# empymod/emg3d

Measured on AMD Instinct MI355X. Metric: Mcells/s per multigrid cycle, higher is better.
Workload: dtype c128

## Files before the change

### emg3d_amd/_lib.py

```python
import ctypes
import os

import numpy as np

_HERE = os.path.dirname(os.path.abspath(__file__))
LIB_PATH = os.environ.get("EMG3D_HIP_LIB") or os.path.join(_HERE, "libemg3d_hip.so")
LAB_PATH = os.path.join(_HERE, "libemg3d_hip_lab.so")

c_i64 = ctypes.c_int64
c_int = ctypes.c_int
c_vp = ctypes.c_void_p
c_double = ctypes.c_double
c_dp = ctypes.POINTER(ctypes.c_double)

ABI_VERSION = 111

SIGNATURES = {
    "emg3d_hip_version": (c_int, []),
    "emg3d_hip_device_count": (c_int, [ctypes.POINTER(c_int)]),
    "emg3d_hip_set_device": (c_int, [c_int]),
    "emg3d_hip_device_info": (c_int, [c_int, ctypes.c_char_p, ctypes.POINTER(c_i64), ctypes.POINTER(c_int)]),
    "emg3d_hip_mem_info": (c_int, [c_int, ctypes.POINTER(c_i64), ctypes.POINTER(c_i64)]),
    "emg3d_hip_release_cached": (c_i64, []),
    "emg3d_hip_cached_bytes": (c_i64, []),
    "emg3d_hip_cached_bytes_on": (c_i64, [c_int]),
    "emg3d_mg_placement": (c_int, [c_vp, c_int, ctypes.POINTER(c_int), ctypes.POINTER(c_int), ctypes.POINTER(ctypes.c_float)]),
    "emg3d_amat_x": (c_int, [c_int, c_i64, c_i64, c_i64, c_vp, c_vp, c_vp, c_vp, c_vp, c_vp, c_vp, c_vp, c_vp]),
    "emg3d_get_h_field": (c_int, [c_int, c_i64, c_i64, c_i64, c_vp, c_vp, c_vp, c_vp, c_vp, c_vp, c_double, c_double]),
    "emg3d_gauss_seidel": (c_int, [c_int, c_int, c_i64, c_i64, c_i64, c_vp, c_vp, c_vp, c_vp, c_vp, c_vp,
                                   c_vp, c_vp, c_vp, c_int, c_int]),
    "emg3d_restrict": (c_int, [c_int, c_i64, c_i64, c_i64, c_i64, c_i64, c_i64, c_vp, c_vp, c_vp, c_int]),
    "emg3d_restrict_weights": (c_int, [c_vp, c_vp, c_vp, c_i64, c_vp, c_vp, c_vp, c_i64, c_vp, c_vp, c_vp]),
    "emg3d_solve": (c_int, [c_int, c_vp, c_vp, c_i64]),
    "emg3d_blocks_to_amat": (c_int, [c_int, c_vp, c_vp, c_i64, c_vp, c_vp, c_vp, c_i64, c_i64]),
    "emg3d_prolongation": (c_int, [c_int, c_i64, c_i64, c_i64, c_vp, c_vp, c_vp, c_vp, c_vp, c_vp, c_int]),
    "emg3d_restrict_model": (c_int, [c_int, c_i64, c_i64, c_i64, c_vp, c_vp, c_int]),
    "emg3d_sweep_plan": (c_int, [c_int, c_i64, c_i64, c_i64, c_int, c_int, c_int, c_int, ctypes.c_char_p, ctypes.POINTER(c_i64)]),
    "emg3d_sweep_fuse_plan": (c_int, [c_int, c_i64, c_i64, c_i64, c_int, c_int, c_int, c_int, c_int, c_int, c_int, c_i64, ctypes.POINTER(c_i64),
                                      ctypes.POINTER(c_i64), c_i64]),
    "emg3d_mg_create": (c_int, [ctypes.POINTER(c_vp), c_int, c_i64, c_i64, c_i64, c_vp, c_vp, c_vp, c_vp,
                                c_vp, c_vp, c_vp, c_vp, c_int]),
    "emg3d_mg_destroy": (None, [c_vp]),
    "emg3d_mg_create_sv": (c_int, [ctypes.POINTER(c_vp), c_int, c_i64, c_i64, c_i64, c_vp, c_vp, c_vp, c_vp,
                                   c_vp, c_vp, c_vp, c_vp, c_double, c_double, c_int]),
    "emg3d_mg_create_vs": (c_int, [ctypes.POINTER(c_vp), c_int, c_i64, c_i64, c_i64, c_vp, c_vp, c_vp, c_vp,
                                   c_vp, c_vp, c_vp, c_vp, c_vp, c_double, c_double, c_int, c_int]),
    "emg3d_mg_create_vse": (c_int, [ctypes.POINTER(c_vp), c_int, c_i64, c_i64, c_i64, c_vp, c_vp, c_vp, c_vp,
                                    c_vp, c_vp, c_vp, c_vp, c_vp, c_vp, c_double, c_double, c_double, c_int, c_int]),
    "emg3d_mg_set_smu0_eps": (c_int, [c_vp, c_double, c_double, c_double]),
    "emg3d_mg_set_model": (c_int, [c_vp, c_int, c_vp, c_vp, c_vp]),
    "emg3d_mg_get_sigma": (c_int, [c_vp, c_int, c_vp]),
    "emg3d_mg_set_sfield_vector": (c_int, [c_vp, c_vp, c_double, c_double]),
    "emg3d_mg_set_sfield_dipole": (c_int, [c_vp, c_vp, c_vp, c_int, c_int, c_vp]),
    "emg3d_source_field": (c_int, [c_int, c_i64, c_i64, c_i64, c_vp, c_vp, c_vp, c_vp, c_vp, c_vp, c_int, c_vp, c_vp]),
    "emg3d_mg_prepare": (c_int, [c_vp, c_int, c_int]),
    "emg3d_mg_set_trace": (c_int, [c_vp, c_int]),
    "emg3d_mg_get_trace": (c_int, [c_vp, c_int, c_vp, c_vp, c_vp]),
    "emg3d_mg_set_params": (c_int, [c_vp, c_int, c_int, c_int, c_int, c_int, c_vp, c_int]),
    "emg3d_mg_set_sfield": (c_int, [c_vp, c_vp]),
    "emg3d_mg_set_efield": (c_int, [c_vp, c_vp]),
    "emg3d_mg_get_efield": (c_int, [c_vp, c_vp]),
    "emg3d_mg_get_residual": (c_int, [c_vp, c_vp]),
    "emg3d_mg_get_hfield": (c_int, [c_vp, c_int, c_double, c_double, c_vp]),
    "emg3d_interp3d": (c_int, [c_int, c_i64, c_i64, c_i64, c_vp, c_vp, c_vp, c_vp, c_i64, c_vp, c_int, c_int, c_double,
                               c_double, c_vp]),
    "emg3d_get_receiver_response": (c_int, [c_int, c_i64, c_i64, c_i64, c_vp, c_vp, c_vp, c_vp, c_vp, c_int, c_i64,
                                            c_vp, c_vp, c_vp]),
    "emg3d_mg_get_receiver_response": (c_int, [c_vp, c_int, c_int, c_double, c_double, c_i64, c_vp, c_vp, c_vp]),
    "emg3d_edges2cellaverages": (c_int, [c_int, c_i64, c_i64, c_i64, c_vp, c_vp, c_vp, c_vp, c_vp]),
    "emg3d_mg_gradient": (c_int, [c_vp, c_int, c_double, c_double, c_vp]),
    "emg3d_mg_gradient3": (c_int, [c_vp, c_int, c_double, c_double, c_vp, c_vp, c_vp]),
    "emg3d_mg_grad_acc_reset": (c_int, [c_vp]),
    "emg3d_mg_grad_acc_add": (c_int, [c_vp, c_int, c_double, c_double, c_vp]),
    "emg3d_mg_grad_acc_get": (c_int, [c_vp, c_vp]),
    "emg3d_mg_grad_acc3_reset": (c_int, [c_vp]),
    "emg3d_mg_grad_acc3_add": (c_int, [c_vp, c_int, c_double, c_double, c_vp]),
    "emg3d_mg_grad_acc3_get": (c_int, [c_vp, c_vp, c_vp, c_vp]),
    "emg3d_cells2edges": (c_int, [c_int, c_i64, c_i64, c_i64, c_vp, c_vp, c_vp, c_vp, c_vp, c_vp, c_vp]),
    "emg3d_mg_jvec_source": (c_int, [c_vp, c_int, c_double, c_double, c_vp, c_vp, c_vp]),
    "emg3d_mg_jvec_source_b": (c_int, [c_vp, c_int, c_double, c_double, c_vp, c_vp, c_vp, c_vp]),
    "emg3d_mg_get_receiver_response_linear": (c_int, [c_vp, c_i64, c_vp, c_vp, c_vp]),
    "emg3d_mg_set_receiver_adjoint": (c_int, [c_vp, c_i64, c_vp, c_vp, c_vp, c_int]),
    "emg3d_mg_get_receiver_response_linear_h": (c_int, [c_vp, c_double, c_double, c_i64, c_vp, c_vp, c_vp]),
    "emg3d_mg_set_receiver_adjoint_ex": (c_int, [c_vp, c_int, c_int, c_double, c_double, c_i64, c_vp, c_vp, c_vp, c_int]),
    "emg3d_mg_set_receiver_adjoint_b": (c_int, [c_vp, c_int, c_int, c_double, c_double, c_i64, c_vp, c_vp, c_vp, c_vp, c_int]),
    "emg3d_receiver_adjoint": (c_int, [c_int, c_i64, c_i64, c_i64, c_vp, c_vp, c_vp, c_vp, c_int, c_int, c_double, c_double,
                                       c_i64, c_vp, c_vp, c_vp, c_vp]),
    "emg3d_volume_average_weights": (c_int, [c_vp, c_i64, c_vp, c_i64, c_vp, c_vp, c_vp, c_vp, c_vp]),
    "emg3d_volume_average": (c_int, [c_int, c_i64, c_i64, c_i64, c_vp, c_vp, c_vp, c_vp, c_i64, c_i64, c_i64, c_vp, c_vp,
                                     c_vp, c_vp, c_vp]),
    "emg3d_interp3d_grid": (c_int, [c_int, c_i64, c_i64, c_i64, c_vp, c_vp, c_vp, c_vp, c_i64, c_vp, c_i64, c_vp, c_i64,
                                    c_vp, c_int, c_int, c_double, c_double, c_vp]),
    "emg3d_mg_set_batch": (c_int, [c_vp, c_int]),
    "emg3d_mg_get_batch": (c_int, [c_vp]),
    "emg3d_mg_select": (c_int, [c_vp, c_int]),
    "emg3d_mg_set_mask": (c_int, [c_vp, c_vp]),
    "emg3d_mg_residual_norm": (c_int, [c_vp, c_dp]),
    "emg3d_mg_sfield_norm": (c_int, [c_vp, c_dp]),
    "emg3d_mg_smooth": (c_int, [c_vp, c_int, c_int]),
    "emg3d_mg_begin": (c_int, [c_vp, c_int]),
    "emg3d_mg_set_smu0": (c_int, [c_vp, ctypes.c_double, ctypes.c_double]),
    "emg3d_mg_cycle": (c_int, [c_vp, c_int, c_int, c_dp]),
    "emg3d_mg_cycle_next": (c_int, [c_vp, c_int, c_int, c_int, c_int, c_dp]),
    "emg3d_mg_cycles": (c_int, [c_vp, c_int, c_vp, c_int, c_vp, c_int, c_vp]),
    "emg3d_mg_efield_devptr": (c_vp, [c_vp]),
    "emg3d_mg_sfield_devptr": (c_vp, [c_vp]),
    "emg3d_mg_stream": (c_vp, [c_vp]),
    "emg3d_mg_nE": (c_i64, [c_vp]),
    "emg3d_mg_sync": (c_int, [c_vp]),
    "emg3d_mg_device_bytes": (c_i64, [c_vp]),
    "emg3d_mg_time_sweep": (c_int, [c_vp, c_int, c_int, ctypes.POINTER(ctypes.c_float)]),
    "emg3d_mg_last_sweep_kernel": (c_int, [c_vp, ctypes.c_char_p]),
    "emg3d_mg_time_residual": (c_int, [c_vp, c_int, ctypes.POINTER(ctypes.c_float)]),
    "emg3d_mg_last_residual_kernel": (c_int, [c_vp, ctypes.c_char_p]),
    "emg3d_mg_amatvec": (c_int, [c_vp, c_vp, c_vp]),
    "emg3d_mg_vec_alloc": (c_int, [c_vp, c_int]),
    "emg3d_mg_vec_set": (c_int, [c_vp, c_int, c_vp]),
    "emg3d_mg_vec_get": (c_int, [c_vp, c_int, c_vp]),
    "emg3d_mg_vec_copy": (c_int, [c_vp, c_int, c_int]),
    "emg3d_mg_vec_axpy": (c_int, [c_vp, c_int, c_double, c_double, c_int]),
    "emg3d_mg_vec_scale": (c_int, [c_vp, c_int, c_double, c_double]),
    "emg3d_mg_vec_dot": (c_int, [c_vp, c_int, c_int, c_dp]),
# ... 45 lines not shown


def load():
    global _lib, _path
    if _lib is None:
        _lib, _path = _open(LIB_PATH), LIB_PATH
    return _lib


def use(path=None):
    global _lib, _path
    prev = _path or LIB_PATH
    want = path or LIB_PATH
    _lib, _path = _open(want), want
    return prev


def check(status, what):
    if status != 0:
        raise HipLibraryError(f"{what} failed with status {status} "
                              f"({'invalid argument' if status < 0 else 'HIP error'})")


def dtype_code(dtype):
    dtype = np.dtype(dtype)
    if dtype == np.complex128:
        return 1
    if dtype == np.float64:
        return 0
    raise TypeError(f"fields must be float64 or complex128, got {dtype}")


def ptr(a):
    return a.ctypes.data_as(c_vp)


def device_count():
    n = c_int(0)
    check(load().emg3d_hip_device_count(ctypes.byref(n)), "emg3d_hip_device_count")
    return n.value


def device_info(device=0):
    name = ctypes.create_string_buffer(256)
    mem = c_i64(0)
    cus = c_int(0)
    check(load().emg3d_hip_device_info(device, name, ctypes.byref(mem), ctypes.byref(cus)),
          "emg3d_hip_device_info")
    return {"name": name.value.decode(), "total_mem": mem.value, "cu_count": cus.value}


def mem_info(device=0):
    fr, tot = c_i64(0), c_i64(0)
    check(load().emg3d_hip_mem_info(device, ctypes.byref(fr), ctypes.byref(tot)), "emg3d_hip_mem_info")
    return {"free": fr.value, "total": tot.value, "pooled": int(load().emg3d_hip_cached_bytes()),
            "pooled_on_device": int(load().emg3d_hip_cached_bytes_on(device))}


def sweep_plan(vnC, direction, dtype=np.complex128, ordering='colour', nsys=1, cu_count=0):
    name = ctypes.create_string_buffer(64)
    info = (c_i64 * 6)()
    check(load().emg3d_sweep_plan(dtype_code(dtype), int(vnC[0]), int(vnC[1]), int(vnC[2]), int(direction),
                                  1 if ordering == 'colour' else 0, int(nsys), int(cu_count), name, info), "emg3d_sweep_plan")
    return {"kernel": name.value.decode(), "lines_per_colour": info[0], "lines_per_wave": info[1], "rounds": info[2],
            "factor_kind": info[3], "split": bool(info[4]), "big_offsets": bool(info[5])}


def sweep_fuse_plan(vnC, direction, npass, dtype=np.complex128, ordering='colour', nsys=1, cu_count=0, own=0, max_seg=0, budget=0):
    info = (c_i64 * 8)()
    cap = (4 + 2 * max(int(npass), 0)) * (max(vnC) + 1)
    ranges = (c_i64 * cap)()
    check(load().emg3d_sweep_fuse_plan(dtype_code(dtype), int(vnC[0]), int(vnC[1]), int(vnC[2]), int(direction),
                                       1 if ordering == 'colour' else 0, int(nsys), int(cu_count), int(npass), int(own), int(max_seg), int(budget),
                                       info, ranges, cap), "emg3d_sweep_fuse_plan")
    out = {"fused": bool(info[0]), "axis": info[1], "nX": info[2], "own": info[3], "nslabs": info[4], "npass": info[5],
           "waves": info[6], "scratch_bytes": info[7], "slabs": []}
    if out["fused"]:
        per = 4 + 2 * int(npass)
        for k in range(info[4]):
            r = ranges[per * k:per * (k + 1)]
            out["slabs"].append({"own": (r[0], r[1]), "edges": (r[2], r[3]),
                                 "live": [(r[4 + 2 * p], r[5 + 2 * p]) for p in range(int(npass))]})
    return out
```

### emg3d_amd/csrc/emg3d_hip.hip

```cpp
#include "../../include/emg3d_hip.h"

#include <cstring>
#include <new>

#include <chrono>
#include "mg.hpp"
#include "receivers.hpp"
#include "source.hpp"
#include "gradient.hpp"
#include "regrid.hpp"

#define EMG3D_HIP_VERSION EMG3D_HIP_ABI_VERSION

namespace {

template <class T>
MG<T>* as(emg3d_mg_t* mg) { return static_cast<MG<T>*>(reinterpret_cast<emg3d_mg*>(mg)); }

static int current_device() { int d = 0; if (hipGetDevice(&d) != hipSuccess) { (void)hipGetLastError(); d = 0; } return d; }

template <class T> static T scalar_of(double re, double im);
template <> double scalar_of<double>(double re, double) { return re; }
template <> c128 scalar_of<c128>(double re, double im) { return mk(re, im); }

// ... 436 lines not shown
    std::vector<double> nodes[3], centers[3];
    for (int a = 0; a < 3; ++a) grid_vectors(hh[a], nC[a], origin ? origin[a] : 0.0, nodes[a], centers[a]);
    const i64 nF = is_electric ? n_edges(nC) : hfield_size(nC);
    T *df = nullptr, *scr = nullptr;
    DEV_ALLOC(df, (size_t)nF * sizeof(T));
    DEV_ALLOC(scr, (size_t)nF * sizeof(T));
    HIP_TRY(hipMemcpy(df, field, (size_t)nF * sizeof(T), hipMemcpyHostToDevice));
    RcvComp<T> comp[3];
    receiver_components<T>(nodes, centers, nC, is_electric != 0, df, comp);
    const int rc = receiver_response_device<T>(nullptr, comp, n, xyz, fac, scr, (T*)resp);
        return rc;
}

template <class T>
int interp3d_host_impl(i64 nx, i64 ny, i64 nz, const double* px, const double* py, const double* pz, const void* values,
                       i64 n, const double* xi, int method, int has_fill, double fill, double cval, void* out) {
    const i64 nn[3] = {nx, ny, nz};
    std::vector<double> pts[3];
    pts[0].assign(px, px + nx); pts[1].assign(py, py + ny); pts[2].assign(pz, pz + nz);
    const i64 tot = nx * ny * nz;
    T *dv = nullptr, *scr = nullptr, *dout = nullptr;
    DEV_ALLOC(dv, (size_t)tot * sizeof(T));
    DEV_ALLOC(scr, (size_t)tot * sizeof(T));
    DEV_ALLOC(dout, (size_t)n * sizeof(T));
    HIP_TRY(hipMemcpy(dv, values, (size_t)tot * sizeof(T), hipMemcpyHostToDevice));
    int rc = interp3d_device<T>(nullptr, dv, nn, 0, 1, nx, nx * ny, pts, n, xi, method, has_fill != 0, fill, cval, nullptr, scr, dout);
    if (rc == 0 && hipMemcpy(out, dout, (size_t)n * sizeof(T), hipMemcpyDeviceToHost) != hipSuccess) rc = (int)hipGetLastError();
        return rc;
}

}

template <class T>
static void* efield_ptr(MG<T>* m) {
    if (hipSetDevice(m->device) != hipSuccess) { (void)hipGetLastError(); return nullptr; }
    T* p = m->sel_e();
    m->check_launch();
    return m->err ? nullptr : (void*)p;
}

template <class T>
static int sweep_plan_impl(i64 nx, i64 ny, i64 nz, int dir, int order, int nsys, int cu_count, char* name, int64_t* info) {
    SweepKnobs K;
    if (cu_count > 0) K.simds = 4 * (i64)cu_count;
    else sweep_device_knobs<T>(K, current_device());
    K.order = order; K.nsys = nsys;
    const SweepPlan p = plan_sweep(K, SweepShape{{nx, ny, nz}, (int)sizeof(T)}, dir - 1);
    memcpy(name, p.name, sizeof p.name);
    info[0] = p.nmax; info[1] = p.lpw; info[2] = p.rounds; info[3] = p.fac_kind; info[4] = p.split ? 1 : 0; info[5] = p.big ? 1 : 0;
    return 0;
}

template <class T>
static int fuse_plan_impl(i64 nx, i64 ny, i64 nz, int dir, int order, int nsys, int cu_count, int npass, int own, int max_seg, i64 budget, int64_t* info,
                          int64_t* ranges, i64 nranges) {
    SweepKnobs K;
    if (cu_count > 0) K.simds = 4 * (i64)cu_count;
    else sweep_device_knobs<T>(K, current_device());
    K.order = order; K.nsys = nsys;
    if (own > 0) K.fuse_own = own;
    if (max_seg > 0) K.fuse_max_seg = max_seg;
    if (budget > 0) K.fuse_max_bytes = budget;
    const SweepShape G{{nx, ny, nz}, (int)sizeof(T)};
    const FusePlan f = plan_fuse(K, G, dir - 1, npass);
    int P, Q;
    sweep_axes(dir - 1, P, Q);
    info[0] = f.fused ? 1 : 0; info[1] = f.axis ? Q : P; info[2] = f.g.nX; info[3] = f.g.own; info[4] = f.g.nslabs; info[5] = f.g.npass;
    info[6] = f.nw; info[7] = f.scratch_bytes;
    if (!f.fused || !ranges) return 0;
    const i64 per = 4 + 2 * (i64)npass;
    if (nranges < per * f.g.nslabs) return -2;
    for (int k = 0; k < f.g.nslabs; ++k) {
        int64_t* r = ranges + per * k;
        r[0] = fuse_x0(f.g, k); r[1] = fuse_x1(f.g, k);
        i64 a = -1, b = -1;
        for (int j = 0; j <= f.g.nX; ++j) if (fuse_owner(f.g, j) == k) { if (a < 0) a = j; b = j + 1; }
        r[2] = a; r[3] = b;
        for (int p = 0; p < npass; ++p) { r[4 + 2 * p] = fuse_lo(f.g, k, p); r[5 + 2 * p] = fuse_hi(f.g, k, p); }
    }
    return 0;
}

template <class T>
static int jvec_stage(MG<T>* m, const double* const hv[3], const double* dv[3]) {
    Level<T>& L = *m->lv0;
    double* stage = reinterpret_cast<double*>(L.r);
    const i64 n = L.nCells;
    int used = 0;
    for (int c = 0; c < 3; ++c) {
        dv[c] = nullptr;
        if (!hv[c]) continue;
        for (int q = 0; q < c; ++q) if (hv[q] == hv[c]) dv[c] = dv[q];
        if (dv[c]) continue;
        double* d = stage + (i64)used++ * n;
        HIP_TRY(hipMemcpyAsync(d, hv[c], (size_t)n * sizeof(double), hipMemcpyHostToDevice, m->stream));
        dv[c] = d;
    }
    return 0;
}

template <class T>
static int jvec_source_impl(MG<T>* m, int efield_vec, double smu0_re, double smu0_im, const double* vx, const double* vy,
                            const double* vz) {
    if (sizeof(T) == 8 && smu0_im != 0.0) return -2;
    HIP_TRY(hipSetDevice(m->device));
    Level<T>& L = *m->lv0;
    const T* fwd = m->vec(efield_vec);
    if (!fwd || efield_vec < 0) return -2;
    const double* hv[3] = {vx, vy, vz};
    const double* dv[3];
    { const int st = jvec_stage<T>(m, hv, dv); if (st) return st; }
    T* s = m->sel_s();
    if (m->broken) return (int)hipErrorOutOfMemory;
    hipLaunchKernelGGL(k_jvec_source<T>, dim3((unsigned)((L.nE + 255) / 256)), dim3(256), 0, m->stream, L.nC[0], L.nC[1], L.nC[2],
                       L.fl, fwd, smu0_re, smu0_im, dv[0], dv[1], dv[2], (const double*)L.h[0], (const double*)L.h[1],
                       (const double*)L.h[2], s, L.nE);
    m->source_changed();
    m->lv0->s_dense = true;
    m->check_launch();
    return finish(m);
}

template <class T>
static int jvec_source_b_impl(MG<T>* m, int fwd_bvec, double smu0_re, double smu0_im, const double* vx, const double* vy,
                              const double* vz, const int32_t* use) {
    if (sizeof(T) == 8 && smu0_im != 0.0) return -2;
    HIP_TRY(hipSetDevice(m->device));
    Level<T>& L = *m->lv0;
    if (fwd_bvec < 0 || fwd_bvec >= (int)m->bvecs.size()) return -2;
    const T* fwd = m->bvecs[(size_t)fwd_bvec];
    unsigned long long bits = 0;
    for (int b = 0; b < m->nsys; ++b) if (use[b]) bits |= 1ull << b;
    if (!bits) return 0;
    const double* hv[3] = {vx, vy, vz};
    const double* dv[3];
    { const int st = jvec_stage<T>(m, hv, dv); if (st) return st; }
    if (m->broken) return (int)hipErrorOutOfMemory;
    hipLaunchKernelGGL(k_jvec_source_b<T>, dim3((unsigned)((L.nE + 255) / 256)), dim3(256), 0, m->stream, L.nC[0], L.nC[1], L.nC[2],
                       L.fl, fwd, m->nsys, bits, smu0_re, smu0_im, dv[0], dv[1], dv[2], (const double*)L.h[0], (const double*)L.h[1],
                       (const double*)L.h[2], L.s, L.nE);
    m->source_changed();
    m->lv0->s_dense = true;
    m->check_launch();
    return finish(m);
}

static int gradient_impl(emg3d_mg_t* mg, int efield_vec, double smu0_re, double smu0_im, double* gx, double* gy, double* gz) {
    const bool split = gy != nullptr;
    DISPATCH(mg, {
        HIP_TRY(hipSetDevice(m->device));
        Level<T>& L = *m->lv0;
        const T* fwd = m->vec(efield_vec);
        if (!fwd || efield_vec == -2) return -2;
        double* dg = reinterpret_cast<double*>(L.r);
        const i64 n = L.nCells;
        const unsigned blocks = (unsigned)((n + 255) / 256);
        const T* bwd = m->sel_e();
        if (m->broken) return (int)hipErrorOutOfMemory;
        if (split)
            hipLaunchKernelGGL((k_gradient<T, true>), dim3(blocks), dim3(256), 0, m->stream, L.nC[0], L.nC[1], L.nC[2], L.fl, fwd, bwd,
                               smu0_re, smu0_im, (const double*)L.h[0], (const double*)L.h[1], (const double*)L.h[2], dg, dg + n, dg + 2 * n);
        else
            hipLaunchKernelGGL((k_gradient<T, false>), dim3(blocks), dim3(256), 0, m->stream, L.nC[0], L.nC[1], L.nC[2], L.fl, fwd, bwd,
                               smu0_re, smu0_im, (const double*)L.h[0], (const double*)L.h[1], (const double*)L.h[2], dg, (double*)nullptr,
                               (double*)nullptr);
        m->check_launch();
// ... 171 lines not shown
    const hipError_t e = hipMemGetInfo(&fr, &tot);
    (void)hipSetDevice(prev);
    if (e != hipSuccess) { (void)hipGetLastError(); return (int)e; }
    if (free_bytes) *free_bytes = (int64_t)fr;
    if (total_bytes) *total_bytes = (int64_t)tot;
    return 0;
}

int emg3d_amat_x(int dtype, int64_t nx, int64_t ny, int64_t nz, void* r, const void* e, const void* eta_x,
                 const void* eta_y, const void* eta_z, const double* zeta, const double* hx,
                 const double* hy, const double* hz) {
    return dtype ? amat_x_impl<c128>(nx, ny, nz, r, e, eta_x, eta_y, eta_z, zeta, hx, hy, hz)
                 : amat_x_impl<double>(nx, ny, nz, r, e, eta_x, eta_y, eta_z, zeta, hx, hy, hz);
}

int emg3d_get_h_field(int dtype, int64_t nx, int64_t ny, int64_t nz, void* hfield, const void* efield,
                      const double* zeta, const double* hx, const double* hy, const double* hz,
                      double smu0_re, double smu0_im) {
    if (nx < 1 || ny < 1 || nz < 1 || !hfield || !efield || !hx || !hy || !hz) return -2;
    if (smu0_re == 0.0 && smu0_im == 0.0) return -2;
    if (!dtype && smu0_im != 0.0) return -2;
    return dtype ? hfield_impl<c128>(nx, ny, nz, hfield, efield, zeta, hx, hy, hz, smu0_re, smu0_im)
                 : hfield_impl<double>(nx, ny, nz, hfield, efield, zeta, hx, hy, hz, smu0_re, smu0_im);
}

int emg3d_gauss_seidel(int dtype, int dir, int64_t nx, int64_t ny, int64_t nz, void* e, const void* s,
                       const void* eta_x, const void* eta_y, const void* eta_z, const double* zeta,
                       const double* hx, const double* hy, const double* hz, int nu, int order) {
    return dtype ? gs_impl<c128>(dir, nx, ny, nz, e, s, eta_x, eta_y, eta_z, zeta, hx, hy, hz, nu, order)
                 : gs_impl<double>(dir, nx, ny, nz, e, s, eta_x, eta_y, eta_z, zeta, hx, hy, hz, nu, order);
}

int emg3d_restrict(int dtype, int64_t nx, int64_t ny, int64_t nz, int64_t cnx, int64_t cny, int64_t cnz,
                   void* cr, const void* r, const double* const* w, int sc_dir) {
    return dtype ? restrict_impl<c128>(nx, ny, nz, cnx, cny, cnz, cr, r, w, sc_dir)
                 : restrict_impl<double>(nx, ny, nz, cnx, cny, cnz, cr, r, w, sc_dir);
}

int emg3d_restrict_weights(const double* vectorN, const double* vectorCC, const double* h, int64_t nh,
                           const double* cvectorN, const double* cvectorCC, const double* ch, int64_t n,
                           double* wl, double* w0, double* wr) {
    if (n < 2 || nh < 2) return -2;
    restrict_weights_host(vectorN, vectorCC, h, nh, cvectorN, cvectorCC, ch, n, wl, w0, wr);
    return 0;
}

int emg3d_solve(int dtype, void* amat, void* bvec, int64_t n) {
    if (n < 1) return -2;
    return dtype ? solve_impl<c128>(amat, bvec, n) : solve_impl<double>(amat, bvec, n);
}

int emg3d_blocks_to_amat(int dtype, void* amat, void* bvec, int64_t n, const void* middle, const double* left,
                         const void* rhs, int64_t im, int64_t nC) {
    return dtype ? b2a_impl<c128>(amat, bvec, n, middle, left, rhs, im, nC)
                 : b2a_impl<double>(amat, bvec, n, middle, left, rhs, im, nC);
}

int emg3d_prolongation(int dtype, int64_t nx, int64_t ny, int64_t nz, const double* hx, const double* hy,
                       const double* hz, const double* origin, void* e, const void* ce, int sc_dir) {
    return dtype ? prolong_impl<c128>(nx, ny, nz, hx, hy, hz, origin, e, ce, sc_dir)
                 : prolong_impl<double>(nx, ny, nz, hx, hy, hz, origin, e, ce, sc_dir);
}

int emg3d_restrict_model(int is_complex, int64_t nx, int64_t ny, int64_t nz, void* cparam, const void* param,
                         int sc_dir) {
    return is_complex ? restrict_model_impl<c128>(nx, ny, nz, cparam, param, sc_dir)
                      : restrict_model_impl<double>(nx, ny, nz, cparam, param, sc_dir);
}

int emg3d_sweep_plan(int dtype, int64_t nx, int64_t ny, int64_t nz, int dir, int order, int nsys, int cu_count, char* name,
                     int64_t* info) {
    if (nx < 2 || ny < 2 || nz < 2 || dir < 1 || dir > 3 || order < 0 || order > 1 || nsys < 1 || nsys > 64 || !name || !info) return -2;
    return dtype ? sweep_plan_impl<c128>(nx, ny, nz, dir, order, nsys, cu_count, name, info)
                 : sweep_plan_impl<double>(nx, ny, nz, dir, order, nsys, cu_count, name, info);
}

int emg3d_sweep_fuse_plan(int dtype, int64_t nx, int64_t ny, int64_t nz, int dir, int order, int nsys, int cu_count, int npass, int own,
                          int max_seg, int64_t budget, int64_t* info, int64_t* ranges, int64_t nranges) {
    if (nx < 2 || ny < 2 || nz < 2 || dir < 1 || dir > 3 || order < 0 || order > 1 || nsys < 1 || nsys > 64 || npass < 0 || !info) return -2;
    return dtype ? fuse_plan_impl<c128>(nx, ny, nz, dir, order, nsys, cu_count, npass, own, max_seg, budget, info, ranges, nranges)
                 : fuse_plan_impl<double>(nx, ny, nz, dir, order, nsys, cu_count, npass, own, max_seg, budget, info, ranges, nranges);
}

int emg3d_mg_create(emg3d_mg_t** out, int dtype, int64_t nx, int64_t ny, int64_t nz, const double* hx,
                    const double* hy, const double* hz, const double* origin, const void* eta_x,
                    const void* eta_y, const void* eta_z, const double* zeta, int device) {
    if (!out) return -1;
    return dtype ? create_impl<c128>(out, 1, nx, ny, nz, hx, hy, hz, origin, eta_x, eta_y, eta_z, zeta, device)
                 : create_impl<double>(out, 0, nx, ny, nz, hx, hy, hz, origin, eta_x, eta_y, eta_z, zeta, device);
}

int emg3d_mg_create_sv(emg3d_mg_t** out, int dtype, int64_t nx, int64_t ny, int64_t nz, const double* hx,
                       const double* hy, const double* hz, const double* origin, const double* sv_x,
                       const double* sv_y, const double* sv_z, const double* zeta, double smu0_re,
                       double smu0_im, int device) {
    if (!out || !sv_x) return -1;
    return dtype ? create_impl<c128>(out, 1, nx, ny, nz, hx, hy, hz, origin, sv_x, sv_y, sv_z, zeta, device, true, smu0_re, smu0_im)
                 : create_impl<double>(out, 0, nx, ny, nz, hx, hy, hz, origin, sv_x, sv_y, sv_z, zeta, device, true, smu0_re, smu0_im);
}

int emg3d_mg_create_vs(emg3d_mg_t** out, int dtype, int64_t nx, int64_t ny, int64_t nz, const double* hx,
                       const double* hy, const double* hz, const double* origin, const double* sigma_x,
                       const double* sigma_y, const double* sigma_z, const double* vol, const double* zeta,
                       double smu0_re, double smu0_im, int map, int device) {
    if (!out || !sigma_x || !vol) return -1;
    if (map < 0 || map >= EMG_MAP_CODES) return -2;
    if (dtype ? smu0_re != 0.0 : smu0_im != 0.0) return -2;
    return dtype ? create_impl<c128>(out, 1, nx, ny, nz, hx, hy, hz, origin, sigma_x, sigma_y, sigma_z, zeta, device, true, smu0_re, smu0_im, vol, map)
                 : create_impl<double>(out, 0, nx, ny, nz, hx, hy, hz, origin, sigma_x, sigma_y, sigma_z, zeta, device, true, smu0_re, smu0_im, vol, map);
}

int emg3d_mg_create_vse(emg3d_mg_t** out, int dtype, int64_t nx, int64_t ny, int64_t nz, const double* hx,
                        const double* hy, const double* hz, const double* origin, const double* sigma_x,
                        const double* sigma_y, const double* sigma_z, const double* vol, const double* zeta,
                        const double* epsilon_r, double smu0_re, double smu0_im, double seps0, int map, int device) {
    if (!out || !sigma_x || !vol || !epsilon_r) return -1;
    if (map < 0 || map >= EMG_MAP_CODES) return -2;
    if (dtype ? smu0_re != 0.0 : smu0_im != 0.0) return -2;
    return dtype ? create_impl<c128>(out, 1, nx, ny, nz, hx, hy, hz, origin, sigma_x, sigma_y, sigma_z, zeta, device, true, smu0_re, smu0_im, vol, map, epsilon_r, seps0)
                 : create_impl<double>(out, 0, nx, ny, nz, hx, hy, hz, origin, sigma_x, sigma_y, sigma_z, zeta, device, true, smu0_re, smu0_im, vol, map, epsilon_r, seps0);
}

void emg3d_mg_destroy(emg3d_mg_t* mg) {
    if (!mg) return;
    const bool broken = reinterpret_cast<emg3d_mg*>(mg)->dtype ? as<c128>(mg)->broken : as<double>(mg)->broken;
    delete reinterpret_cast<emg3d_mg*>(mg);
    if (broken) (void)hipGetLastError();
}

int emg3d_mg_set_params(emg3d_mg_t* mg, int cycle, int nu_init, int nu_pre, int nu_coarse, int nu_post,
                        const int* clevel, int order) {
    if (cycle != 'V' && cycle != 'W' && cycle != 'F') return -2;
    if (order != 0 && order != 1) return -2;
    DISPATCH(mg, {
        bool same = m->cycle == cycle && m->nu_init == nu_init && m->nu_pre == nu_pre && m->nu_coarse == nu_coarse &&
                    m->nu_post == nu_post && m->order == order;
        if (clevel) for (int q = 0; q < 4; ++q) same = same && m->clevel[q] == clevel[q];
        if (!same) m->drop_graphs();
        m->cycle = cycle; m->cycmax = (cycle == 'V') ? 1 : 2;
        m->entry_cm = 0;
        m->nu_init = nu_init; m->nu_pre = nu_pre; m->nu_coarse = nu_coarse; m->nu_post = nu_post;
        if (clevel) {
            bool changed = false;
            for (int q = 0; q < 4; ++q) { if (m->clevel[q] != clevel[q]) changed = true; m->clevel[q] = clevel[q]; }
            if (changed) m->hier.clear();
        }
        if (m->order != order) {
            HIP_TRY(hipSetDevice(m->device));
            m->e_to_ref(*m->lv0);
            m->check_launch();
            m->order = order;
            m->forget_factors();
        }
        return 0;
    });
}

int emg3d_mg_set_smu0(emg3d_mg_t* mg, double smu0_re, double smu0_im) {
    DISPATCH(mg, {
        HIP_TRY(hipSetDevice(m->device));
        if (sizeof(T) == 8 && smu0_im != 0.0) return -2;
        if (sizeof(T) == 16 && m->volw && smu0_re != 0.0) return -2;
        if (m->epsr) return -7;
        const int st = m->set_smu0(scalar_of<T>(smu0_re, smu0_im));
        if (st) return st;
        return finish(m);
// ... 690 lines not shown
```

### emg3d_amd/csrc/mg.hpp

```cpp
#pragma once
#include <algorithm>
#include <cmath>
#include <cstdlib>
#include <cstring>
#include <map>
#include <memory>
#include <mutex>
#include <chrono>
#include <vector>

#include "common.hpp"
#include "smooth.hpp"
#include "stencil.hpp"
#include "gradient.hpp"
#include "smooth_qpl.hpp"
#include "smooth_qc.hpp"
#include "smooth_thm.hpp"
#include "smooth_tha.hpp"
#include "sweep_launch.hpp"
#include "sweep_plan.hpp"

template <class T>
struct Level {
    i64 nC[3];
    i64 nE, nCells;
    FieldLayout fl;
    CellLayout cl;
    std::vector<double> h_host[3], nodes[3], centers[3];
    double* h[3] = {nullptr, nullptr, nullptr};
    double* ih[3] = {nullptr, nullptr, nullptr};
    T* eta[3] = {nullptr, nullptr, nullptr};
    double* zeta = nullptr;
    unsigned char* sflag[3] = {nullptr, nullptr, nullptr};
    bool sflag_valid[3] = {false, false, false};
    bool s_dense = false;
    bool zeta_sep = false;
    T *s = nullptr, *e = nullptr, *r = nullptr;
    T *eT = nullptr, *sT = nullptr;
    T* etaT[3] = {nullptr, nullptr, nullptr};
    double* zetaT = nullptr;
    bool sT_valid = false;
    FieldLayout flT;
    CellLayout clT;
    T *eW[2] = {nullptr, nullptr}, *sW[2] = {nullptr, nullptr};
    double* zetaW[2] = {nullptr, nullptr};
    bool sW_valid[2] = {false, false};
    int e_home = 0;
    T* fac[3] = {nullptr, nullptr, nullptr};
    void* qd[3][4] = {{nullptr, nullptr, nullptr, nullptr}, {nullptr, nullptr, nullptr, nullptr}, {nullptr, nullptr, nullptr, nullptr}};
    unsigned qdn[3][4] = {{0, 0, 0, 0}, {0, 0, 0, 0}, {0, 0, 0, 0}};
    T* fz[3] = {nullptr, nullptr, nullptr};
    i64 fz_n[3] = {0, 0, 0};
    FusePlan fuse[3];
    int fuse_key[3] = {-1, -1, -1};
    std::vector<int> passes[3];
    i64 fac_lines[3] = {0, 0, 0};
    i64 fac_mid[3] = {0, 0, 0};
    int fac_kind[3] = {0, 0, 0};
    SweepPlan plan[3];
    int plan_key[3] = {-1, -1, -1};
};

struct Transfer {
    int sc = -1;
    int co[3] = {0, 0, 0};
    double* w[3][3] = {{nullptr, nullptr, nullptr}, {nullptr, nullptr, nullptr}, {nullptr, nullptr, nullptr}};
    int* pidx[3] = {nullptr, nullptr, nullptr};
    double* pwt[3] = {nullptr, nullptr, nullptr};
};

template <class T>
struct Hierarchy {
    std::vector<std::shared_ptr<Level<T>>> lv;
    std::vector<Transfer> tr;
};

class DevicePool {
    std::mutex mu;
    struct Parked { void* p; int tag; };
    std::multimap<std::pair<int, size_t>, Parked> free_blocks;
    size_t held = 0, cap;
public:
    DevicePool() {
        const char* g = getenv("EMG3D_POOL_GB");
        cap = (size_t)((g ? atof(g) : 96.0) * (double)((size_t)1 << 30));
    }
    void* take(int device, size_t nb, int tag = 0, bool* hit = nullptr) {
        std::lock_guard<std::mutex> lk(mu);
        if (hit) *hit = false;
        auto rng = free_blocks.equal_range({device, nb});
        if (rng.first == rng.second) return nullptr;
        auto pick = rng.second;
        for (auto it = rng.first; it != rng.second; ++it) if (it->second.tag == tag) { pick = it; break; }
        if (pick == rng.second && tag != 0)
            for (auto it = rng.first; it != rng.second; ++it) if (it->second.tag == 0) { pick = it; break; }
        if (pick == rng.second) pick = rng.first;
        if (hit) *hit = tag != 0 && pick->second.tag == tag;
        void* p = pick->second.p;
        free_blocks.erase(pick);
        held -= nb;
        return p;
    }
    bool give(int device, void* p, size_t nb, int tag = 0) {
        std::lock_guard<std::mutex> lk(mu);
        if (held + nb > cap) return false;
        free_blocks.insert({{device, nb}, Parked{p, tag}});
        held += nb;
        return true;
    }
    size_t release_all() {
        std::lock_guard<std::mutex> lk(mu);
        const size_t n = held;
        int cur = 0;
        (void)hipGetDevice(&cur);
        for (auto& kv : free_blocks) {
            if (kv.first.first < 0) { (void)hipHostFree(kv.second.p); continue; }
            (void)hipSetDevice(kv.first.first); (void)hipFree(kv.second.p);
        }
        for (auto& kv : free_streams) { (void)hipSetDevice(kv.first); (void)hipStreamDestroy(kv.second); }
        free_streams.clear();
        (void)hipSetDevice(cur);
        free_blocks.clear();
        held = 0;
        return n;
    }
    size_t bytes_held() { std::lock_guard<std::mutex> lk(mu); return held; }
    size_t bytes_held_on(int device) {
        std::lock_guard<std::mutex> lk(mu);
        size_t n = 0;
        for (auto& kv : free_blocks) if (kv.first.first == device) n += kv.first.second;
        return n;
    }
    std::multimap<int, hipStream_t> free_streams;
    hipStream_t take_stream(int device) {
        {
// ... 915 lines not shown
                a.rs.off[c] = (unsigned)a.fl.off[ax[c]];
                for (int d = 0; d < 3; ++d) a.rs.st[c][d] = (unsigned)a.fl.st[ax[c]][ax[d]];
            }
        }
        a.qd = nullptr; a.qdn = 0;
        a.fe = nullptr; a.fnE = 0; a.fax = a.fnX = a.fown = a.fns = a.fnp = 0; a.fseq = 0;
        for (int c = 0; c < 4; ++c) { a.fqd[c] = nullptr; a.fqdn[c] = 0; }
        a.qpl = P.NW; a.qM = P.M; a.seg = P.seg; a.qlpw = 0;
        a.tha = P.helpers;
        a.mode = 0; a.cP = a.cQ = 0; a.cntA = a.cntB = 0; a.t = a.jQ0 = a.cnt = 0;
        a.bt = sweep ? batch(L) : Batch();
    }

    void ensure_factor(Level<T>& L, int dir) {
        const SweepPlan& P = plan(L, dir);
        if (P.xt) ensure_transposed_model(L);
        if (L.fac[dir]) return;
        L.fac_lines[dir] = (L.nC[dir == 0 ? 1 : 0] - 1) * (L.nC[dir == 2 ? 1 : 2] - 1);
        L.fac[dir] = dalloc<T>(L.fac_lines[dir] * P.fac_entries);
        L.fac_mid[dir] = P.mid;
        L.fac_kind[dir] = P.fac_kind;
        if (P.fac_kind == 3) thm_attrs();
        compute_factor(L, dir);
    }
    void compute_factor(Level<T>& L, int dir) {
        LineArgs<T> a;
        line_args(L, dir, a, false);
        a.fac = L.fac[dir];
        a.fcomp = L.fac_kind[dir] == 4;
        if (L.fac_kind[dir] == 3) {
            a.mid = L.fac_mid[dir];
            const i64 nQ_ = L.nC[a.Q];
            const i64 nmax_ = a.nA[0] * ((nQ_ - 0) / 2);
            a.mode = 3;
            if (nmax_ > 0)
                MG_LAUNCH(k_line_factor_m<T>, dim3((unsigned)((nmax_ + EMG_LINE_BLOCK - 1) / EMG_LINE_BLOCK), 4),
                                   dim3(EMG_LINE_BLOCK), 0, stream, a);
            check_launch();
            return;
        }
        a.mid = L.fac_mid[dir];
        const i64 nQ = L.nC[a.Q];
        const i64 nB[2] = {(nQ - 0) / 2, (nQ - 1) / 2};
        a.mode = 3; a.cP = a.cQ = 0; a.cntA = a.cntB = 0;
        const i64 nmax = a.nA[0] * nB[0];
#ifdef EMG3D_LAB
        if (LAB_ENV("EMG3D_FACTOR_PER_COLOUR", 0)) {
            for (int c = 0; c < 4; ++c) {
                a.mode = 0; a.cP = c & 1; a.cQ = c >> 1; a.cntA = a.nA[a.cP]; a.cntB = nB[a.cQ];
                const i64 n = a.cntA * a.cntB;
                if (n > 0)
                    MG_LAUNCH(k_line_factor<T>, dim3((unsigned)((n + EMG_LINE_BLOCK - 1) / EMG_LINE_BLOCK)),
                                       dim3(EMG_LINE_BLOCK), 0, stream, a);
            }
            check_launch();
            return;
        }
#endif
        if (nmax > 0)
            MG_LAUNCH(k_line_factor<T>, dim3((unsigned)((nmax + EMG_LINE_BLOCK - 1) / EMG_LINE_BLOCK), 4),
                               dim3(EMG_LINE_BLOCK), 0, stream, a);
        check_launch();
    }

    unsigned xcd_grid(i64 nb) const { return (unsigned)(xcd_map ? ((nb + 7) / 8) * 8 : nb); }
    unsigned rp_grid(i64 nt) const { return xcd_grid((nt + EMG_RP_BLOCK - 1) / EMG_RP_BLOCK); }
    void ensure_qdesc(Level<T>& L, int dir) {
        const SweepPlan& P = plan(L, dir);
        if (!P.qdesc || L.qd[dir][0] || L.qdn[dir][0] == ~0u) return;
        L.qdn[dir][0] = ~0u;
        if (!L.fac[dir]) return;
        LineArgs<T> a;
        line_args(L, dir, a, true);
        const i64 lpg = 16 / a.seg;
        a.bt = Batch();
        for (int c = 0; c < 4; ++c) {
            a.mode = 0; a.cP = c & 1; a.cQ = c >> 1;
            a.cntA = a.nA[a.cP]; a.cntB = a.nB2[a.cQ];
            a.rs.slot0 = (unsigned)a.base[c];
            const i64 n = a.cntA * a.cntB;
            if (n <= 0) continue;
            const unsigned grid = xcd_grid((n + lpg - 1) / lpg);
            const i64 nthreads = (i64)grid * 64;
            void* tab = try_alloc<char>(nthreads * a.qM * (3 * 16 + 8 * 16));
            if (!tab) return;
            a.qd = tab; a.qdn = (unsigned)nthreads;
            if (!broken) qpl_launch<T>(1, a.qM, false, 1, false, dim3(grid), stream, a);
            L.qd[dir][c] = tab; L.qdn[dir][c] = (unsigned)nthreads;
        }
        check_launch();
    }
    char sweep_name[64] = "";
    char res_name[64] = "";
    int thm_lifo = (int)LAB_ENV("EMG3D_THM_LIFO", 0);
    void thm_attrs() {
#ifdef EMG3D_LAB
        static bool done[64] = {false};
        if (device < 0 || device >= 64 || done[device]) return;
        done[device] = true;
        thm_lifo_attrs<T>();
#endif
    }
    void launch_sweep(const SweepPlan& P, const LineArgs<T>& a, i64 n) {
        if (log_launches) fprintf(stderr, "[sweep] nC %lld %lld %lld L %d lines %lld kernel %s split %d\n", (long long)a.nC[0], (long long)a.nC[1], (long long)a.nC[2], a.L, (long long)n,
                                  P.name, a.split);
        memcpy(sweep_name, P.name, sizeof sweep_name);
        if (broken) return;
        switch (P.family) {
        case SweepFamily::tha: {
            const size_t dyn = P.helpers == 2 ? tha_lds_bytes<T, 2>((int)a.nC[a.L]) : tha_lds_bytes<T, 3>((int)a.nC[a.L]);
            tha_launch<T>(P.helpers, a.zsep != 0, bgrid(xcd_grid((n + THA_LPW - 1) / THA_LPW)), dyn, stream, a);
            break;
        }
        case SweepFamily::thm: {
            const i64 npairs = (n + P.inst_lpw - 1) / P.inst_lpw;
            thm_launch<T>(P.stages, P.inst_lpw, thm_lifo != 0, a.zsep != 0, bgrid(rp_grid(npairs * 128)), stream, a);
            break;
        }
        case SweepFamily::qpl:
        case SweepFamily::qpl_chain: {
            const i64 lpg = (16 * P.NW) / P.seg;
            qpl_launch<T>(P.NW, P.M, false, (P.NW == 1 && a.qd) ? 2 : 0, P.family == SweepFamily::qpl_chain,
                          bgrid(xcd_grid((n + lpg - 1) / lpg)), stream, a);
            break;
        }
        case SweepFamily::qc:
        case SweepFamily::qc_big: {
            LineArgs<T> b = a;
            b.qlpw = P.inst_lpw == 16 ? sweep_balanced_lpw(knobs, n * nsys) : P.inst_lpw;
            qc_launch<T>(P.stages, P.inst_lpw, a.zsep != 0, P.big, bgrid(rp_grid(((n + b.qlpw - 1) / b.qlpw) * 64)), stream, b);
            break;
        }
        case SweepFamily::rp: {
            const unsigned g = rp_grid(((n + P.inst_lpw - 1) / P.inst_lpw) * 64);
            if (P.inst_lpw == 8) hipLaunchKernelGGL((k_line_sweep_rp<T, 8>), bgrid(g), dim3(EMG_RP_BLOCK), 0, stream, a);
            else if (P.inst_lpw == 12) hipLaunchKernelGGL((k_line_sweep_rp<T, 12>), bgrid(g), dim3(EMG_RP_BLOCK), 0, stream, a);
            else hipLaunchKernelGGL((k_line_sweep_rp<T, 4>), bgrid(g), dim3(EMG_RP_BLOCK), 0, stream, a);
            break;
        }
        case SweepFamily::tpl:
            hipLaunchKernelGGL(k_line_sweep<T>, bgrid_y((unsigned)((n + EMG_LINE_BLOCK - 1) / EMG_LINE_BLOCK)), dim3(EMG_LINE_BLOCK), 0, stream, a);
            break;
        }
    }

    void prepare_work(Level<T>& L, int dir) {
        ensure_sflags(L, dir);
        if (home_on(L) || home_lvl(L)) ensure_work(L, 1);
        if (split_on(L)) ensure_work(L, (dir == 0) ? 0 : 1);
        else if (plan(L, dir).xt) ensure_transposed_model(L);
    }
    void to_work(Level<T>& L, int dir) {
        ensure_sflags(L, dir);
        if (split_on(L)) {
            const int w = (dir == 0) ? 0 : 1;
            ensure_work(L, w);
            if (home_lvl(L)) {
                if (w == 0) {
                    if (!L.sW_valid[0]) { convert_field(L, L.sW[0], L.sW[1], 2, true); L.sW_valid[0] = true; }
                    convert_field(L, L.eW[0], L.eW[1], 2, true);
                }
                return;
            }
            if (!L.sW_valid[w]) { convert_field(L, L.sW[w], L.s, w, true); L.sW_valid[w] = true; }
            if (!home_on(L)) convert_field(L, L.eW[w], L.e, w, true);
            else {
                e_to_w1(L);
// ... 69 lines not shown
            if (placed[w] || dir < 0 || !L.eW[w] || !L.sW[w] || !L.fac[dir]) continue;
            placed[w] = true;
            if (w == 1) e_to_ref(L);
            if (!L.sW_valid[w]) { convert_field(L, L.sW[w], L.s, w, true); L.sW_valid[w] = true; }
            ensure_sflags(L, dir);
            const i64 n = (i64)nsys * L.nE;
            PlaceRec& R = place_rec[w];
            R = PlaceRec();
            T* cands[PLACE_MAX];
            cands[0] = L.eW[w];
            int best = 0;
            float worst = 0.f;
            const int nt = std::min<int>(place_tries, PLACE_MAX);
            for (int k = 0; k < nt; ++k) {
                T* c = (k == 0) ? cands[0] : try_alloc<T>(n);
                if (!c) break;
                cands[k] = c;
                hipMemsetAsync(c, 0, (size_t)n * sizeof(T), stream);
                L.eW[w] = c;
                if (k == 0) (void)time_sweeps(L, dir, 1);
                const float ms = time_sweeps(L, dir, place_reps);
                R.ms[k] = ms;
                R.tries = k + 1;
                if (ms < 0.f) break;
                if (ms < R.ms[best]) best = k;
                worst = std::max(worst, ms);
                if ((double)R.ms[best] * place_gap < (double)worst) break;
            }
            if (R.ms[best] < 0.f) best = 0;
            R.kept = best;
            L.eW[w] = cands[best];
            block_tag[cands[best]] = 1 + w;
            for (int k = 0; k < R.tries; ++k) if (k != best) release(cands[k]);
            moved |= best != 0;
            if (getenv("EMG3D_LOG_SETUP")) {
                fprintf(stderr, "[place] working copy %d (%s-lines, %.0f MB): kept candidate %d of %d;", w, dir == 0 ? "x" : dir == 1 ? "y" : "z",
                        (double)n * sizeof(T) / 1048576.0, best, R.tries);
                for (int k = 0; k < R.tries; ++k) fprintf(stderr, " %.3f", R.ms[k]);
                fprintf(stderr, " ms per sweep\n");
            }
        }
        if (moved) drop_graphs();
        check_launch();
    }

    void colour_passes(Level<T>& L, int dir, int nu, std::vector<int>& seq) {
        int Pa, Qa;
        sweep_axes(dir, Pa, Qa);
        const i64 nP = L.nC[Pa], nQ = L.nC[Qa];
        int iback = 0, last_c = -1;
        seq.clear();
        for (int it = 0; it < nu; ++it) {
            iback = 1 - iback;
            for (int ch = 0; ch < 4; ++ch) {
                const int c = iback ? colour_perm_b[ch] : colour_perm[ch];
                if (skip_idempotent && c == last_c) continue;
                last_c = c;
                if (((nP - (c & 1)) / 2) * ((nQ - (c >> 1)) / 2) <= 0) continue;
                seq.push_back(c);
            }
        }
    }
    const FusePlan& ensure_fuse(Level<T>& L, int dir, int nu) {
        const int key = nu * 256 + order + 2 * nsys;
        if (L.fuse_key[dir] == key) return L.fuse[dir];
        FusePlan& F = L.fuse[dir];
        F = FusePlan();
        L.fuse_key[dir] = key;
        L.passes[dir].clear();
        if (order != 1) return F;
        colour_passes(L, dir, nu, L.passes[dir]);
        const std::vector<int>& seq = L.passes[dir];
        plan(L, dir);
        F = plan_fuse(knobs, SweepShape{{L.nC[0], L.nC[1], L.nC[2]}, (int)sizeof(T)}, dir, (int)seq.size());
        if (!F.fused) return F;
        for (int c : seq) if (!L.qd[dir][c]) { F.fused = false; return F; }
        const i64 need = (i64)nsys * F.g.nslabs * L.nE;
        if (L.fz_n[dir] < need) {
            T* z = try_alloc<T>(need);
            if (!z) { F.fused = false; return F; }
            if (L.fz[dir]) release(L.fz[dir]);
            L.fz[dir] = z; L.fz_n[dir] = need;
        }
        return F;
    }
    void smooth_fused(Level<T>& L, int dir, const SweepPlan& P, const FusePlan& F, const std::vector<int>& seq, const LineArgs<T>& a) {
        LineArgs<T> b = a;
        b.mode = 0; b.xcd = 0;
        b.fe = L.fz[dir]; b.fnE = L.nE; b.fax = F.axis;
        b.fnX = F.g.nX; b.fown = F.g.own; b.fns = F.g.nslabs; b.fnp = F.g.npass;
        b.fseq = 0;
        for (int p = 0; p < F.g.npass; ++p) b.fseq |= (unsigned long long)seq[(size_t)p] << (4 * p);
        for (int c = 0; c < 4; ++c) { b.fqd[c] = L.qd[dir][c]; b.fqdn[c] = L.qd[dir][c] ? L.qdn[dir][c] : 0u; }
        if (log_launches) fprintf(stderr, "[sweep] nC %lld %lld %lld L %d lines %lld kernel %s split %d fused passes %d slabs %d own %d\n", (long long)a.nC[0],
                                  (long long)a.nC[1], (long long)a.nC[2], a.L, (long long)a.nLinesTot, P.name, a.split, F.g.npass, F.g.nslabs, F.g.own);
        memcpy(sweep_name, P.name, sizeof sweep_name);
        if (broken) return;
        qpl_fused_launch<T>(P.family == SweepFamily::qpl_chain, bgrid((unsigned)F.g.nslabs), stream, b);
        ScatterArgs sa;
        sa.nE = L.nE; sa.g = F.g;
        int Pa, Qa;
        sweep_axes(dir, Pa, Qa);
        sa.ax = F.axis ? Qa : Pa;
        for (int c = 0; c < 3; ++c) {
            sa.off[c] = L.fl.off[c];
            sa.d0[c] = (unsigned)((c == 0) ? L.nC[0] : L.nC[0] + 1); sa.d1[c] = (unsigned)((c == 1) ? L.nC[1] : L.nC[1] + 1);
        }
        hipLaunchKernelGGL(k_scatter_slabs<T>, dim3((unsigned)((L.nE + EMG_BLOCK - 1) / EMG_BLOCK), (unsigned)nsys), dim3(EMG_BLOCK), 0, stream,
                           a.e, (const T*)L.fz[dir], sa, a.bt);
    }

    void smooth_line(Level<T>& L, int dir, int nu, bool conv_in = true, bool conv_out = true) {
        if (nu <= 0) return;
        ensure_factor(L, dir);
        ensure_qdesc(L, dir);
        const FusePlan& F = ensure_fuse(L, dir, nu);
        if (dry) { prepare_work(L, dir); return; }
        if (conv_in) to_work(L, dir);
        ensure_sflags(L, dir);
        LineArgs<T> a;
        line_args(L, dir, a, true);
        const SweepPlan& P = plan(L, dir);
        const i64 nP = L.nC[a.P], nQ = L.nC[a.Q];
        const i64 nB[2] = {(nQ - 0) / 2, (nQ - 1) / 2};
        if (order == 1) {
            if (F.fused) smooth_fused(L, dir, P, F, L.passes[dir], a);
            else for (int c : L.passes[dir]) {
                a.mode = 0; a.cP = c & 1; a.cQ = c >> 1;
                a.cntA = a.nA[a.cP]; a.cntB = nB[a.cQ];
                a.rs.slot0 = (unsigned)a.base[c];
                a.qd = L.qd[dir][c]; a.qdn = (L.qd[dir][c] ? L.qdn[dir][c] : 0u);
                launch_sweep(P, a, a.cntA * a.cntB);
            }
            nu = 0;
        }
        int iback = 0;
        for (int it = 0; it < nu; ++it) {
            iback = 1 - iback;
            {
                const i64 tmin = 3, tmax = (nP - 1) + 2 * (nQ - 1);
                if (lex_loop && a.qpl && a.qM == 1 && a.seg <= 16) {
                    LineArgs<T> b = a;
                    b.mode = 2; b.t = tmin; b.jQ0 = tmax; b.cnt = iback; b.xcd = 0;
                    const i64 maxn = std::min<i64>(nQ - 1, (nP - 1) / 2 + 1), quads = maxn * a.seg;
                    const int lnw = quads <= 16 ? 1 : quads <= 32 ? 2 : quads <= 64 ? 4 : 8;
                    if (!broken) qpl_launch<T>(lnw, 1, true, 0, false, bgrid(1), stream, b);
                    sweep_kernel_name(sweep_name, sizeof sweep_name, SweepFamily::qpl, (int)sizeof(T), lnw, 1);
                    continue;
                }
                for (i64 th = tmin; th <= tmax; ++th) {
                    const i64 tt = iback ? tmax - (th - tmin) : th;
                    i64 lo = tt - (nP - 1);
                    i64 jQ0 = lo <= 0 ? 1 : (lo + 1) / 2;
                    if (jQ0 < 1) jQ0 = 1;
                    i64 jQ1 = (tt - 1) / 2;
                    if (jQ1 > nQ - 1) jQ1 = nQ - 1;
                    const i64 n = jQ1 - jQ0 + 1;
                    if (n <= 0) continue;
                    a.mode = 1; a.t = tt; a.jQ0 = jQ0; a.cnt = n;
                    launch_sweep(P, a, n);
                }
            }
        }
        if (conv_out) from_work(L, dir);
        check_launch();
    }

    void smooth_point(Level<T>& L, int nu) {
        if (dry) return;
        if (&L == lv0.get()) e_to_ref(L);
        const bool hl = home_lvl(L) && L.e_home == 1;
        if (hl) { convert_field(L, L.e, L.eW[1], 1, false); convert_field(L, L.s, L.sW[1], 1, false); }
        PointArgs<T> a;
        for (int q = 0; q < 3; ++q) { a.nC[q] = L.nC[q]; a.eta[q] = L.eta[q]; a.h[q] = L.h[q]; a.ih[q] = L.ih[q]; }
        a.fl = L.fl; a.e = L.e; a.s = L.s; a.zeta = L.zeta; a.bt = batch(L);
        a.col = 0; a.t = 0; a.cnt[0] = a.cnt[1] = a.cnt[2] = 0;
        int iback = 0;
        int last_c = -1;
        for (int it = 0; it < nu; ++it) {
            iback = 1 - iback;
            if (order == 1) {
// ... 162 lines not shown
        Level<T>& L = *lv0;
        if (L.sT && !L.sT_valid) { convert_field(L, L.sT, L.s, -1, true); L.sT_valid = true; }
        for (int w = 0; w < 2; ++w)
            if (L.sW[w] && !L.sW_valid[w]) { convert_field(L, L.sW[w], L.s, w, true); L.sW_valid[w] = true; }
        for (int d = 0; d < 3; ++d)
            if (L.sflag[d]) ensure_sflags(L, d);
    }

    void prepare(int g, int lr_dir) {
        if (!use_graph) { dry = true; cycle0_eager(g, lr_dir, 0); dry = false; place_level0(lr_dir); return; }
        cycle0(g, lr_dir, -1);
    }

    void cycle0(int g, int lr_dir, int slot) {
        if (!use_graph || trace) {
            if (slot >= 0) {
                if (placement_pending(lr_dir)) prepare(g, lr_dir);
                cycle0_eager(g, lr_dir, slot);
            }
            return;
        }
        const int key = (g * 8 + lr_dir) * 4 + entry_cm;
        auto it = graphs.find(key);
        if (it != graphs.end() && slot < 0) return;
        const int home_in = (home_on(*lv0) && current_lr_dir(lr_dir, lv0->nC) != 0) ? 1 : 0;
        if (it == graphs.end()) {
            const bool tlog = getenv("EMG3D_LOG_SETUP") != nullptr;
            auto now = [] { return std::chrono::steady_clock::now(); };
            auto ms = [](auto a, auto b) { return std::chrono::duration<double, std::milli>(b - a).count(); };
            auto t0 = now();
            const size_t nalloc0 = allocs.size();
            dry = true;
            cycle0_eager(g, lr_dir, 0);
            dry = false;
            place_level0(lr_dir);
            const int home_keep = (slot >= 0) ? home_in : lv0->e_home;
            if (slot >= 0) { if (home_in) e_to_w1(*lv0); else e_to_ref(*lv0); }
            else if (home_in) ensure_work(*lv0, 1);
            lv0->e_home = home_in;
            refresh_level0_source();
            if (tlog) hipStreamSynchronize(stream);
            auto t1 = now();
            hipGraph_t graph = nullptr;
            hipGraphExec_t exec = nullptr;
            hipError_t st = hipStreamBeginCapture(stream, hipStreamCaptureModeThreadLocal);
            if (st == hipSuccess) {
                cycle0_eager(g, lr_dir, 0);
                st = hipStreamEndCapture(stream, &graph);
            }
            const int home_out = lv0->e_home;
            lv0->e_home = home_keep;
            auto t2 = now();
            if (st == hipSuccess) st = hipGraphInstantiate(&exec, graph, nullptr, nullptr, 0);
            if (graph) hipGraphDestroy(graph);
            if (tlog) fprintf(stderr, "[setup] key %d: hierarchy+factors %.2f ms (%zu allocations), capture %.2f ms, instantiate %.2f ms\n",
                              key, ms(t0, t1), allocs.size() - nalloc0, ms(t1, t2), ms(t2, now()));
            if (st != hipSuccess || err != 0) {
                (void)hipGetLastError();
                fprintf(stderr, "[emg3d_hip] hipGraph capture failed (%s); using eager launches\n", hipGetErrorString(st));
                use_graph = false;
                err = 0;
                if (slot >= 0) cycle0_eager(g, lr_dir, slot);
                return;
            }
            (void)hipGraphUpload(exec, stream);
            graphs[key] = exec;
            graph_home[key] = std::make_pair(home_in, home_out);
            it = graphs.find(key);
            if (slot < 0) return;
        }
        const std::pair<int, int> hm = graph_home[key];
        if (hm.first) e_to_w1(*lv0); else e_to_ref(*lv0);
        refresh_level0_source();
        hipError_t st = hipGraphLaunch(it->second, stream);
        if (st != hipSuccess && err == 0) err = (int)st;
        lv0->e_home = hm.second;
        if (slot != 0) hipMemcpyAsync(norms + (i64)slot * nsys, norms, (size_t)nsys * sizeof(double), hipMemcpyDeviceToDevice, stream);
    }

    void forget_factors() {
        auto clear = [](Level<T>& L) {
            for (int d = 0; d < 3; ++d) {
                L.fac[d] = nullptr; L.fac_kind[d] = 0; L.plan_key[d] = -1; L.fuse_key[d] = -1;
                for (int c = 0; c < 4; ++c) { L.qd[d][c] = nullptr; L.qdn[d][c] = 0; }
            }
        };
        if (lv0) clear(*lv0);
        for (auto& kv : hier) for (auto& l : kv.second.lv) if (l) clear(*l);
    }

    void drop_graphs() {
        for (auto& kv : graphs) hipGraphExecDestroy(kv.second);
        graphs.clear();
        graph_home.clear();
        graph_seen.clear();
    }
};
```

### emg3d_amd/csrc/smooth.hpp

```cpp
#pragma once
#include "common.hpp"

#define EMG_LINE_BLOCK 64

template <class T>
struct LineArgs {
    int L, P, Q;
    i64 nC[3];
    FieldLayout fl;
    CellLayout cl;
    T* e;
    const T* s;
    const T* eta[3];
    const double* zeta;
    const double* h[3];
    const double* ih[3];
    int split;
    i64 mid;
    int xcd;
    int tile;
    struct Resolved {
        const double *ihL, *ihP, *ihQ;
        const double *hL, *hP, *hQ;
        unsigned nL, csL, csP, csQ;
        unsigned nP, nQ;
        unsigned slot0;
        unsigned off[3], st[3][3];
    } rs;
    Batch bt;
    int qm;
    int qpl;
    int qM, seg;
    const unsigned char* sflag;
    int zsep;
    int qlpw;
    int tha;
    int fcomp;
    T* fac;
    const void* qd;
    unsigned qdn;
    T* fe;
    i64 fnE;
    int fax, fnX, fown, fns, fnp;
    unsigned long long fseq;
    const void* fqd[4];
    unsigned fqdn[4];
    i64 nLinesTot;
    i64 base[4];
    i64 nA[2];
    i64 nB2[2];
    int mode;
    int cP, cQ;
    i64 cntA, cntB;
    i64 t, jQ0, cnt;
};

template <class T>
__device__ __forceinline__ bool line_of_thread(const LineArgs<T>& a, i64& jP, i64& jQ) {
    const i64 idx = (i64)blockIdx.x * blockDim.x + threadIdx.x;
    if (a.mode == 0) {
        if (idx >= a.cntA * a.cntB) return false;
        const i64 b = idx / a.cntA, q = idx - b * a.cntA;
        jP = 1 + a.cP + 2 * q;
        jQ = 1 + a.cQ + 2 * b;
    } else {
        if (idx >= a.cnt) return false;
        jQ = a.jQ0 + idx;
        jP = a.t - 2 * jQ;
    }
    return true;
}

template <class T>
__device__ __forceinline__ i64 line_slot(const LineArgs<T>& a, i64 jP, i64 jQ) {
    const int cP = (int)((jP - 1) & 1), cQ = (int)((jQ - 1) & 1);
    return a.base[cP + 2 * cQ] + ((jP - 1) >> 1) + a.nA[cP] * ((jQ - 1) >> 1);
}

struct LineCoef {
    double QP_Lm[2], PQ_Lm[2];
    double QL_Pm[2], LQ_Pm[2], QL_Pp[2], LQ_Pp[2];
    double PL_Qm[2], LP_Qm[2], PL_Qp[2], LP_Qp[2];
};

__device__ __forceinline__ void line_coef(LineCoef& c, const double z[2][2][2], const double kL[2],
                                          const double kP[2], const double kQ[2]) {
#pragma unroll
    for (int S = 0; S < 2; ++S) {
        c.QP_Lm[S] = kP[S] * (z[0][S][1] + z[0][S][0]);
        c.PQ_Lm[S] = kQ[S] * (z[0][1][S] + z[0][0][S]);
        c.QL_Pm[S] = kL[S] * (z[S][0][1] + z[S][0][0]);
        c.LQ_Pm[S] = kQ[S] * (z[1][0][S] + z[0][0][S]);
        c.QL_Pp[S] = kL[S] * (z[S][1][1] + z[S][1][0]);
        c.LQ_Pp[S] = kQ[S] * (z[1][1][S] + z[0][1][S]);
        c.PL_Qm[S] = kL[S] * (z[S][1][0] + z[S][0][0]);
        c.LP_Qm[S] = kP[S] * (z[1][S][0] + z[0][S][0]);
        c.PL_Qp[S] = kL[S] * (z[S][1][1] + z[S][0][1]);
        c.LP_Qp[S] = kP[S] * (z[1][S][1] + z[0][S][1]);
    }
}

__device__ __forceinline__ void line_left(const LineCoef& c, double ihLm, double a[5], double d[5]) {
    a[0] = 0.0; d[0] = 0.0;
    a[1] = c.QP_Lm[0] * ihLm;
    a[2] = -c.QP_Lm[1] * ihLm;
    a[3] = c.PQ_Lm[0] * ihLm;
    a[4] = -c.PQ_Lm[1] * ihLm;
    d[1] = -c.QL_Pm[0] * ihLm;
    d[2] = -c.QL_Pp[0] * ihLm;
    d[3] = -c.PL_Qm[0] * ihLm;
    d[4] = -c.PL_Qp[0] * ihLm;
}

__host__ __device__ __forceinline__ constexpr int wpk(int r, int c) {
    return r >= c ? r * (r + 1) / 2 + c : c * (c + 1) / 2 + r;
}

template <class T>
__device__ __forceinline__ void apply_sinv(const T f[15], T y[5]) {
    T o[5];
#pragma unroll
    for (int r = 0; r < 5; ++r) {
        T t = f[wpk(r, 0)] * y[0];
#pragma unroll
        for (int c = 1; c < 5; ++c) t += f[wpk(r, c)] * y[c];
        o[r] = t;
    }
#pragma unroll
    for (int r = 0; r < 5; ++r) y[r] = o[r];
}

template <class T>
struct BlockMat {
    T S[5][5];
    double al[5], dl[5];
};

template <class T>
// ... 1092 lines not shown
```

### emg3d_amd/csrc/smooth_qpl.hpp

```cpp
#pragma once
#include "smooth.hpp"
#include "sweep_plan.hpp"


template <int K>
__device__ __forceinline__ double quad_bcast(double v) {
    constexpr int ctrl = K | (K << 2) | (K << 4) | (K << 6);
    int lo = __double2loint(v), hi = __double2hiint(v);
    lo = __builtin_amdgcn_update_dpp(0, lo, ctrl, 0xf, 0xf, false);
    hi = __builtin_amdgcn_update_dpp(0, hi, ctrl, 0xf, 0xf, false);
    return __hiloint2double(hi, lo);
}
template <int K>
__device__ __forceinline__ c128 quad_bcast(c128 v) { return mk(quad_bcast<K>(v.re), quad_bcast<K>(v.im)); }
__device__ __forceinline__ double quad_sum(double v) {
    int lo = __double2loint(v), hi = __double2hiint(v);
    double o = __hiloint2double(__builtin_amdgcn_update_dpp(0, hi, 0xb1, 0xf, 0xf, false),
                                __builtin_amdgcn_update_dpp(0, lo, 0xb1, 0xf, 0xf, false));
    v += o;
    lo = __double2loint(v); hi = __double2hiint(v);
    o = __hiloint2double(__builtin_amdgcn_update_dpp(0, hi, 0x4e, 0xf, 0xf, false),
                         __builtin_amdgcn_update_dpp(0, lo, 0x4e, 0xf, 0xf, false));
    return v + o;
}
__device__ __forceinline__ c128 quad_sum(c128 v) { return mk(quad_sum(v.re), quad_sum(v.im)); }

template <bool UP>
__device__ __forceinline__ double row_shift4(double v) {
    constexpr int ctrl = UP ? 0x114 : 0x104;
    int lo = __double2loint(v), hi = __double2hiint(v);
    lo = __builtin_amdgcn_update_dpp(0, lo, ctrl, 0xf, 0xf, false);
    hi = __builtin_amdgcn_update_dpp(0, hi, ctrl, 0xf, 0xf, false);
    return __hiloint2double(hi, lo);
}
template <bool UP> __device__ __forceinline__ c128 row_shift4(c128 v) { return mk(row_shift4<UP>(v.re), row_shift4<UP>(v.im)); }
template <bool UP> __device__ __forceinline__ double lane_shift4(double v) { return UP ? __shfl_up(v, 4) : __shfl_down(v, 4); }
template <bool UP> __device__ __forceinline__ c128 lane_shift4(c128 v) { return mk(lane_shift4<UP>(v.re), lane_shift4<UP>(v.im)); }

template <class T>
__device__ __forceinline__ void qpl_args_burst(const LineArgs<T>& a) {
    asm volatile("" :: "s"(a.e), "s"(a.s), "s"(a.fac), "s"(a.zeta), "s"(a.rs.ihL), "s"(a.rs.ihP), "s"(a.rs.ihQ), "s"(a.bt.st),
                 "s"(a.bt.mask), "s"(a.bt.n), "s"(a.xcd), "s"(a.mode), "s"(a.cntA), "s"(a.cntB), "s"(a.cP), "s"(a.cQ), "s"(a.seg),
                 "s"(a.rs.nL), "s"(a.rs.csL), "s"(a.rs.csP), "s"(a.rs.csQ), "s"(a.rs.slot0), "s"(a.rs.off[0]), "s"(a.rs.off[1]),
                 "s"(a.rs.off[2]));
    asm volatile("" :: "s"(a.rs.st[0][0]), "s"(a.rs.st[0][1]), "s"(a.rs.st[0][2]), "s"(a.rs.st[1][0]), "s"(a.rs.st[1][1]),
                 "s"(a.rs.st[1][2]), "s"(a.rs.st[2][0]), "s"(a.rs.st[2][1]), "s"(a.rs.st[2][2]), "s"(a.t), "s"(a.jQ0), "s"(a.cnt),
                 "s"(a.rs.nP), "s"(a.rs.nQ), "s"(a.qd), "s"(a.qdn));
}

template <class T, int NW, int M, bool HL = false, int DM = 0, bool CH = false, bool FZ = false>
__global__ __launch_bounds__(64 * NW) void k_line_sweep_qpl(LineArgs<T> a) {
    static_assert(DM == 0 || (!HL && (NW == 1 || FZ)), "descriptors: one wave per workgroup, colour order");
    static_assert(!CH || ((NW == 1 || FZ) && M == 1 && !HL), "chain form: lines inside one wave, one block per quad");
    static_assert(!FZ || (DM == 2 && M == 1 && !HL), "fused passes: descriptors, one block per quad, colour order");
    constexpr int NQ = 16 * NW;
#ifdef EMG3D_LAB
    long long qts[7] = {0, 0, 0, 0, 0, 0, 0};
#define QPL_TS(i) do { if (a.tile & 512) { asm volatile("" ::: "memory"); qts[i] = (long long)__builtin_readcyclecounter(); asm volatile("" ::: "memory"); } } while (0)
#else
#define QPL_TS(i) do {} while (0)
#endif
    QPL_TS(0);
    qpl_args_burst(a);
    QPL_TS(1);
    const int tid = threadIdx.x;
    const int quad = tid >> 2, r = tid & 3;
    const int seg = a.seg;
    const int ch = quad & (seg - 1);
    const int lseg = __builtin_ctz((unsigned)seg);
    const int lpg = NQ >> lseg;
    typedef unsigned int u32;
    EMG_SWEEP_WG(a)
    __shared__ T xb[2][(FZ && CH) ? 1 : NQ][4][5];
    T* const ebase = FZ ? a.fe + ((i64)bsys_ * a.fns + wg) * a.fnE : a.e + boff_;
    const void* qd_ = a.qd;
    u32 qdn_ = a.qdn;
    u32 tix = (u32)wg * (64u * NW) + (u32)tid;
    auto one = [&](const u32 gline, const u32 nlines, const u32 t_, const u32 jQ0_) {
    const bool live = gline < nlines;
    const int nL = (int)a.rs.nL;
    auto ld_d = [](const double* base, u32 idx) -> double { return *reinterpret_cast<const double*>(reinterpret_cast<const char*>(base) + idx * 8u); };
    auto ld_t = [](const T* base, u32 idx) -> T { return *reinterpret_cast<const T*>(reinterpret_cast<const char*>(base) + idx * (u32)sizeof(T)); };
    const T* __restrict__ e = ebase;
    const T* __restrict__ s = (a.s + boff_);
    T Wr[M][5], W0[M][5];
    T b[M][5];
    double av[M][4], dv[M][4];
    bool lastb[M], inl[M];
    u32 dS[M], dS0[M];
    constexpr int QD_U4 = 3, QD_D2 = 8;
    if constexpr (DM == 2) {
        const uint4* const q4 = reinterpret_cast<const uint4*>(qd_);
        const emg_d2* const c2 = reinterpret_cast<const emg_d2*>(q4 + (size_t)(QD_U4 * M) * qdn_);
        uint4 u[M][QD_U4];
        emg_d2 cf[M][QD_D2];
#pragma unroll
        for (int j = 0; j < M; ++j) {
#pragma unroll
            for (int k = 0; k < QD_U4; ++k) u[j][k] = q4[(u32)(QD_U4 * j + k) * qdn_ + tix];
#pragma unroll
            for (int k = 0; k < QD_D2; ++k) cf[j][k] = c2[(u32)(QD_D2 * j + k) * qdn_ + tix];
        }
        QPL_TS(2);
        T E[M][6], S[M], E0[M], S0[M];
#pragma unroll
        for (int j = 0; j < M; ++j) {
            const u32 oE[6] = {u[j][0].x, u[j][0].y, u[j][0].z, u[j][0].w, u[j][1].x, u[j][1].y};
            dS[j] = u[j][1].z; dS0[j] = u[j][2].x;
            inl[j] = (u[j][2].z & 1u) != 0; lastb[j] = (u[j][2].z & 2u) != 0;
            const T* w = a.fac + u[j][2].y;
#pragma unroll
            for (int c = 0; c < 5; ++c) W0[j][c] = w[(u32)(wpk(0, c) * (M * seg))];
#pragma unroll
            for (int c = 0; c < 5; ++c) {
                const int e1 = wpk(1, c), e2 = wpk(2, c), e3 = wpk(3, c), e4 = wpk(4, c);
                const int en = (r == 0) ? e1 : (r == 1) ? e2 : (r == 2) ? e3 : e4;
                Wr[j][c] = w[(u32)(en * (M * seg))];
            }
#pragma unroll
            for (int t = 0; t < 6; ++t) E[j][t] = ld_t(e, oE[t]);
            S[j] = ld_t(s, dS[j]);
            E0[j] = ld_t(e, u[j][1].w);
            S0[j] = ld_t(s, dS0[j]);
        }
#pragma unroll
        for (int j = 0; j < M; ++j) {
            const double cE[6] = {cf[j][0].x, cf[j][0].y, cf[j][1].x, cf[j][1].y, cf[j][2].x, cf[j][2].y};
            av[j][0] = cf[j][3].y; av[j][1] = cf[j][4].x; av[j][2] = cf[j][4].y; av[j][3] = cf[j][5].x;
            dv[j][0] = cf[j][5].y; dv[j][1] = cf[j][6].x; dv[j][2] = cf[j][6].y; dv[j][3] = cf[j][7].x;
            T y = S[j];
#pragma unroll
            for (int t = 0; t < 6; ++t) cmac(y, E[j][t], cE[t]);
            const T bo = lastb[j] ? Zero<T>::v() : y;
            T part = E0[j] * cf[j][3].x;
            part = quad_sum(part);
            b[j][0] = S0[j] + part;
            b[j][1] = quad_bcast<0>(bo); b[j][2] = quad_bcast<1>(bo); b[j][3] = quad_bcast<2>(bo); b[j][4] = quad_bcast<3>(bo);
            if (!inl[j]) {
#pragma unroll
                for (int c = 0; c < 5; ++c) { Wr[j][c] = Zero<T>::v(); W0[j][c] = Zero<T>::v(); }
            }
        }
    } else {
    const u32 gidx = live ? gline : 0u;
    u32 jP, jQ;
    if (a.mode == 0) {
        const u32 cA = (u32)a.cntA;
        const u32 bq = gidx / cA, qq = gidx - bq * cA;
        jP = 1u + (u32)a.cP + 2u * qq;
        jQ = 1u + (u32)a.cQ + 2u * bq;
    } else {
        jQ = jQ0_ + gidx;
        jP = t_ - 2u * jQ;
    }
    const u32 slot = (a.mode == 0) ? a.rs.slot0 + gidx : (u32)line_slot(a, (i64)jP, (i64)jQ);
    const u32 csL = a.rs.csL, csP = a.rs.csP, csQ = a.rs.csQ;
    const double ihP[2] = {ld_d(a.rs.ihP, jP - 1u), ld_d(a.rs.ihP, jP)};
    const double ihQ[2] = {ld_d(a.rs.ihQ, jQ - 1u), ld_d(a.rs.ihQ, jQ)};
    const bool tp = r < 2;
    const int side = r & 1;
    const double sg = side ? -1.0 : 1.0;
    const u32 jA = tp ? jP : jQ, jB = tp ? jQ : jP;
    const u32 acell = jA - 1u + (u32)side;
    const u32 anode = side ? jA + 1u : jA - 1u;
    const u32 oLc = a.rs.off[0], oAc = tp ? a.rs.off[1] : a.rs.off[2], oBc = tp ? a.rs.off[2] : a.rs.off[1];
    const u32 sLL = a.rs.st[0][0];
    const u32 sLA = tp ? a.rs.st[0][1] : a.rs.st[0][2], sLB = tp ? a.rs.st[0][2] : a.rs.st[0][1];
    const u32 sAL = tp ? a.rs.st[1][0] : a.rs.st[2][0];
    const u32 sAA = tp ? a.rs.st[1][1] : a.rs.st[2][2], sAB = tp ? a.rs.st[1][2] : a.rs.st[2][1];
    const u32 sBL = tp ? a.rs.st[2][0] : a.rs.st[1][0];
    const u32 sBA = tp ? a.rs.st[2][1] : a.rs.st[1][2], sBB = tp ? a.rs.st[2][2] : a.rs.st[1][1];
    u32 ob[7], os[7];
    ob[0] = oAc + sAL + acell * sAA + jB * sAB;
    ob[1] = oLc + sLL + anode * sLA + jB * sLB;
    ob[2] = ob[1] - sLL;
    ob[3] = oBc + sBL + anode * sBA + jB * sBB;
    ob[4] = ob[3] - sBB;
    ob[5] = ob[0] + sAB;
    ob[6] = ob[0] - sAB;
    os[0] = sAL; os[1] = sLL; os[2] = sLL; os[3] = sBL; os[4] = sBL; os[5] = sAL; os[6] = sAL;
    const u32 sLP = a.rs.st[0][1], sLQ = a.rs.st[0][2];
    const u32 o0 = oLc + jP * sLP + jQ * sLQ;
    const u32 db0 = (r < 2) ? sLP : sLQ;
    const u32 ob0 = (r & 1) ? o0 - db0 : o0 + db0;
    const int type = tp ? 1 : 2;

    T E[M][6], S[M], E0[M], S0[M];
    u32 dE[M][6], dE0[M], dF[M];
    double f00[M], f10[M], f01[M], f11[M], n0[M], n1[M], ihl0[M], ihl1[M];
#pragma unroll
    for (int j = 0; j < M; ++j) {
        const int i = ch * M + j;
        const int ic = i < nL ? i : nL - 1;
        inl[j] = i < nL;
        lastb[j] = (ic == nL - 1);
        if constexpr (DM == 0) {
            const T* w = a.fac + ((i64)slot * (15 * (M * seg)) + ic);
#pragma unroll
            for (int c = 0; c < 5; ++c) W0[j][c] = w[(u32)(wpk(0, c) * (M * seg))];
#pragma unroll
            for (int c = 0; c < 5; ++c) {
                const int e1 = wpk(1, c), e2 = wpk(2, c), e3 = wpk(3, c), e4 = wpk(4, c);
                const int en = (r == 0) ? e1 : (r == 1) ? e2 : (r == 2) ? e3 : e4;
                Wr[j][c] = w[(u32)(en * (M * seg))];
            }
        } else {
// ... 123 lines not shown
            for (int cc = 0; cc < 4; ++cc) {
                T t = g0 * oG[0][cc];
                cmac(t, g1, oG[1][cc]); cmac(t, g2, oG[2][cc]); cmac(t, g3, oG[3][cc]);
                mG[cc] = t;
            }
        }
    };
    auto compose_c_only = [&](int p, int src) {
        cmac(mc, mG[0], xb[p][src][0][0]); cmac(mc, mG[1], xb[p][src][1][0]);
        cmac(mc, mG[2], xb[p][src][2][0]); cmac(mc, mG[3], xb[p][src][3][0]);
    };
    int p = 0;

    auto fwd_row = [&](int j) {
        T t = Wr[j][0] * b[j][0];
#pragma unroll
        for (int c = 1; c < 5; ++c) cmac(t, Wr[j][c], b[j][c]);
        mc = t;
#pragma unroll
        for (int k = 0; k < 4; ++k) {
            T g = Zero<T>::v();
            cmsc(g, Wr[j][0], av[j][k]);
            cmsc(g, Wr[j][k + 1], dv[j][k]);
            mG[k] = g;
        }
    };
    fwd_row(0);
    T u[4];
    if constexpr (CH) {
        auto from_below = [&](T v) -> T { return seg == 4 ? row_shift4<true>(v) : lane_shift4<true>(v); };
        T zc = mc;
#pragma unroll 1
        for (int st = 1; st < seg; ++st) {
            const T up = from_below(zc);
            T t0 = mc, t1 = mG[1] * quad_bcast<1>(up);
            cmac(t0, mG[0], quad_bcast<0>(up)); cmac(t1, mG[3], quad_bcast<3>(up)); cmac(t0, mG[2], quad_bcast<2>(up));
            zc = (ch > 0) ? t0 + t1 : mc;
        }
        const T up = from_below(zc);
        u[0] = quad_bcast<0>(up); u[1] = quad_bcast<1>(up); u[2] = quad_bcast<2>(up); u[3] = quad_bcast<3>(up);
        if (ch == 0) { u[0] = Zero<T>::v(); u[1] = Zero<T>::v(); u[2] = Zero<T>::v(); u[3] = Zero<T>::v(); }
    } else {
#pragma unroll
    for (int j = 1; j < M; ++j) {
        publish(p);
        sync();
        fwd_row(j);
        compose_with(p, quad);
        p ^= 1;
    }
#pragma unroll 1
    for (int st = 1; st < seg; st <<= 1) {
        publish(p);
        sync();
        if (ch >= st) { if (2 * st < seg) compose_with(p, quad - st); else compose_c_only(p, quad - st); }
        p ^= 1;
    }
    publish(p);
    sync();
#pragma unroll
    for (int k = 0; k < 4; ++k) u[k] = (ch > 0) ? xb[p][quad - 1][k][0] : Zero<T>::v();
    p ^= 1;
    }
    T z0[M], zr[M];
#pragma unroll
    for (int j = 0; j < M; ++j) {
        T y[5];
        y[0] = b[j][0];
#pragma unroll
        for (int k = 0; k < 4; ++k) {
            cmsc(y[0], u[k], av[j][k]);
            T t = b[j][k + 1];
            cmsc(t, u[k], dv[j][k]);
            y[k + 1] = t;
        }
        z0[j] = W0[j][0] * y[0];
        zr[j] = Wr[j][0] * y[0];
#pragma unroll
        for (int c = 1; c < 5; ++c) { cmac(z0[j], W0[j][c], y[c]); cmac(zr[j], Wr[j][c], y[c]); }
        if (j + 1 < M) { u[0] = quad_bcast<0>(zr[j]); u[1] = quad_bcast<1>(zr[j]); u[2] = quad_bcast<2>(zr[j]); u[3] = quad_bcast<3>(zr[j]); }
    }

    QPL_TS(4);
    auto bwd_row = [&](int j) {
        const double ar = (r == 0) ? av[j][0] : (r == 1) ? av[j][1] : (r == 2) ? av[j][2] : av[j][3];
        const double dr = (r == 0) ? dv[j][0] : (r == 1) ? dv[j][1] : (r == 2) ? dv[j][2] : dv[j][3];
        T g = z0[j] * ar;
        cmac(g, zr[j], dr);
        mc = g;
#pragma unroll
        for (int l = 0; l < 4; ++l) {
            T h = Zero<T>::v();
            cmsc(h, W0[j][l + 1], ar);
            cmsc(h, Wr[j][l + 1], dr);
            mG[l] = h;
        }
    };
    bwd_row(M - 1);
    T v[4];
    if constexpr (CH) {
        auto from_above = [&](T w) -> T { return seg == 4 ? row_shift4<false>(w) : lane_shift4<false>(w); };
        T vc = mc;
        const bool inner = ch + 1 < seg;
#pragma unroll 1
        for (int st = 1; st < seg; ++st) {
            const T dn = from_above(vc);
            T t0 = mc, t1 = mG[1] * quad_bcast<1>(dn);
            cmac(t0, mG[0], quad_bcast<0>(dn)); cmac(t1, mG[3], quad_bcast<3>(dn)); cmac(t0, mG[2], quad_bcast<2>(dn));
            vc = inner ? t0 + t1 : mc;
        }
        const T dn = from_above(vc);
        v[0] = quad_bcast<0>(dn); v[1] = quad_bcast<1>(dn); v[2] = quad_bcast<2>(dn); v[3] = quad_bcast<3>(dn);
        if (!inner) { v[0] = Zero<T>::v(); v[1] = Zero<T>::v(); v[2] = Zero<T>::v(); v[3] = Zero<T>::v(); }
    } else {
#pragma unroll
    for (int j = M - 2; j >= 0; --j) {
        publish(p);
        sync();
        bwd_row(j);
        compose_with(p, quad);
        p ^= 1;
    }
#pragma unroll 1
    for (int st = 1; st < seg; st <<= 1) {
        publish(p);
        sync();
        if (ch + st < seg) { if (2 * st < seg) compose_with(p, quad + st); else compose_c_only(p, quad + st); }
        p ^= 1;
    }
    publish(p);
    sync();
#pragma unroll
    for (int k = 0; k < 4; ++k) v[k] = (ch + 1 < seg) ? xb[p][quad + 1][k][0] : Zero<T>::v();
    }
    QPL_TS(5);
    T* eo = ebase;
#pragma unroll
    for (int j = M - 1; j >= 0; --j) {
        T x0 = z0[j], xr = zr[j];
#pragma unroll
        for (int l = 0; l < 4; ++l) { cmsc(x0, W0[j][l + 1], v[l]); cmsc(xr, Wr[j][l + 1], v[l]); }
        const int i = ch * M + j;
        if (live && inl[j]) {
            if (r == 0) eo[dS0[j]] = x0;
            if (!lastb[j]) eo[dS[j]] = xr;
        }
        if (j > 0) {
            const double ar = (r == 0) ? av[j][0] : (r == 1) ? av[j][1] : (r == 2) ? av[j][2] : av[j][3];
            const double dr = (r == 0) ? dv[j][0] : (r == 1) ? dv[j][1] : (r == 2) ? dv[j][2] : dv[j][3];
            T vr = x0 * ar;
            cmac(vr, xr, dr);
            v[0] = quad_bcast<0>(vr); v[1] = quad_bcast<1>(vr); v[2] = quad_bcast<2>(vr); v[3] = quad_bcast<3>(vr);
        }
    }
    QPL_TS(6);
    };

    if constexpr (FZ) {
        const FuseGeom g{a.fnX, a.fown, a.fns, a.fnp};
        const int k = (int)wg;
        {
            T* __restrict__ dst = ebase;
            const T* __restrict__ src = a.e + boff_;
            const int ra = fuse_lo(g, k, 0) - 1, rb = fuse_hi(g, k, 0) + 1;
            const int X = a.fax ? 2 : 1;
            const u32 nO = a.fax ? a.rs.nP : a.rs.nQ;
#pragma unroll
            for (int c = 0; c < 3; ++c) {
                const u32 dL = a.rs.nL + (c != 0 ? 1u : 0u), dX = (u32)g.nX + (c != X ? 1u : 0u), dO = nO + ((c == 0 || c == X) ? 1u : 0u);
                const int rbc = rb < (int)dX - 1 ? rb : (int)dX - 1;
                if (rbc < ra) continue;
                const u32 w = (u32)(rbc - ra + 1);
                const u32 stL = a.rs.st[c][0], stX = a.fax ? a.rs.st[c][2] : a.rs.st[c][1], stO = a.fax ? a.rs.st[c][1] : a.rs.st[c][2];
                const bool xf = stX < stL;
                const u32 n0 = xf ? w : dL, n1 = xf ? dL : w, tot = n0 * n1 * dO;
                for (u32 idx = (u32)tid; idx < tot; idx += 64u * NW) {
                    const u32 t = idx / n0, i0 = idx - t * n0, i2 = t / n1, i1 = t - i2 * n1;
                    const u32 iX = (u32)ra + (xf ? i0 : i1), iL = xf ? i1 : i0;
                    const u32 off = a.rs.off[c] + iL * stL + iX * stX + i2 * stO;
                    dst[off] = src[off];
                }
            }
        }
        __threadfence_block();
        __syncthreads();
        const u32 lslot = (u32)(quad >> lseg), wslot0 = (u32)(((tid >> 6) * 16) >> lseg);
        for (int p = 0; p < g.npass; ++p) {
            const int c = (int)((a.fseq >> (4 * p)) & 3ull);
            const int cP = c & 1, cQ = c >> 1;
            const u32 cA = (u32)a.nA[cP], cB = (u32)a.nB2[cQ];
            const int cX = a.fax ? cQ : cP;
            const u32 qa = (u32)(fuse_lo(g, k, p) - cX) >> 1, qb = (u32)(fuse_hi(g, k, p) + 1 - cX) >> 1;
            const u32 nx = qb > qa ? qb - qa : 0u;
            const u32 nloc = nx * (a.fax ? cA : cB);
            qd_ = a.fqd[c]; qdn_ = a.fqdn[c];
            for (u32 base = 0; base < nloc; base += (u32)lpg) {
                if (base + wslot0 < nloc) {
                    const u32 m = base + lslot;
                    const bool lv = m < nloc;
                    const u32 mm = lv ? m : base + wslot0;
                    u32 qq, bq;
                    if (a.fax == 0) { bq = mm / nx; qq = qa + (mm - bq * nx); }
                    else { const u32 t = mm / cA; qq = mm - t * cA; bq = qa + t; }
                    const u32 gl = bq * cA + qq;
                    tix = ((gl >> (4 - lseg)) << 6) + ((((gl & ((16u >> lseg) - 1u)) << lseg) + (u32)ch) << 2) + (u32)r;
                    one(lv ? 0u : 1u, 1u, 0u, 0u);
                }
            }
            __threadfence_block();
            __syncthreads();
        }
    } else if constexpr (!HL) {
        one((u32)wg * (u32)lpg + (u32)(quad >> lseg), (u32)((a.mode == 0) ? a.cntA * a.cntB : a.cnt), (u32)a.t, (u32)a.jQ0);
#ifdef EMG3D_LAB
        if ((a.tile & 512) && blockIdx.x == 0 && threadIdx.x == 0) {
            asm volatile("s_waitcnt vmcnt(0)" ::: "memory");
            const long long tend = (long long)__builtin_readcyclecounter();
            printf("[qpl<%d,%d> seg %d lines %lld] args %lld loads issued %lld loads in + coefficients %lld forward %lld backward %lld stores issued %lld stores done %lld (cycles after entry)\n",
                   NW, M, seg, (long long)(a.cntA * a.cntB), qts[1] - qts[0], qts[2] - qts[0], qts[3] - qts[0], qts[4] - qts[0], qts[5] - qts[0], qts[6] - qts[0], tend - qts[0]);
        }
#endif
    } else {
        const int nPm = (int)a.rs.nP - 1, nQm = (int)a.rs.nQ - 1;
        const int tmin = (int)a.t, tmax = (int)a.jQ0;
        for (int th = tmin; th <= tmax; ++th) {
            const int tt = a.cnt ? tmax - (th - tmin) : th;
            const int lo = tt - nPm;
            int jq0 = lo <= 0 ? 1 : (lo + 1) / 2;
            if (jq0 < 1) jq0 = 1;
            int jq1 = (tt - 1) / 2;
            if (jq1 > nQm) jq1 = nQm;
            const int n = jq1 - jq0 + 1;
            for (int base = 0; base < n; base += lpg) {
                one((u32)(quad >> lseg), (u32)min(n - base, lpg), (u32)tt, (u32)(jq0 + base));
                __threadfence_block();
                __syncthreads();
            }
        }
    }
#undef QPL_TS
}
```

### emg3d_amd/csrc/sweep_launch.hpp

```cpp
#pragma once
#include "smooth.hpp"
#include "stencil.hpp"

template <class T> void qc_launch(int stages, int lpw, bool zsep, bool big, dim3 grid, hipStream_t st, const LineArgs<T>& a);

template <class T> void thm_launch(int stages, int lpw, bool lifo, bool zsep, dim3 grid, hipStream_t st, const LineArgs<T>& a);
template <class T> void thm_lifo_attrs();

template <class T> void tha_launch(int helpers, bool zsep, dim3 grid, size_t dyn_lds, hipStream_t st, const LineArgs<T>& a);
template <class T> bool tha_attrs(int max_dyn_lds);

template <class T> void qpl_launch(int nw, int m, bool hl, int dm, bool chain, dim3 grid, hipStream_t st, const LineArgs<T>& a);
template <class T> void qpl_fused_launch(bool chain, dim3 grid, hipStream_t st, const LineArgs<T>& a);

template <class T> void residual_launch(int mode, int kz, dim3 grid, hipStream_t st, const ResidualArgs<T>& a);
```

### emg3d_amd/csrc/sweep_plan.hpp

```cpp
#pragma once
#include <algorithm>
#include <cstdint>
#include <cstdio>
#include <cstdlib>

typedef int64_t i64;

#ifndef LAB_ENV
#ifdef EMG3D_LAB
inline long long lab_env_(const char* name, long long def) { const char* v = getenv(name); return v ? atoll(v) : def; }
inline int lab_env_ch_(const char* name) { const char* v = getenv(name); return v ? v[0] : 0; }
#define LAB_ENV(name, def) lab_env_(name, (long long)(def))
#define LAB_ENV_CH(name) lab_env_ch_(name)
#else
#define LAB_ENV(name, def) ((long long)(def))
#define LAB_ENV_CH(name) 0
#endif
#endif

constexpr int SWEEP_THA_LPW = 8, SWEEP_THA_RING = 8, SWEEP_THA_MAX_DYN_LDS = 140 * 1024, SWEEP_THA_STATIC_LDS = 18 * 1024;
inline i64 sweep_tha_lds_bytes(i64 nL, int tsize) {
    return (2 * SWEEP_THA_RING * 5 + 2 * ((nL + 1) / 2 + 2)) * (5 * SWEEP_THA_LPW) * (i64)tsize;
}

struct SweepKnobs {
    i64 simds = 1024;
    i64 lds_limit = 160 * 1024;
    bool tha_lds_granted = true;
    int order = 1, nsys = 1;
    int batch_tune = getenv("EMG3D_BATCH_TUNE") ? atoi(getenv("EMG3D_BATCH_TUNE")) : 0;

    int sweep_kernel = LAB_ENV_CH("EMG3D_SWEEP") == 't' ? 1 : 0;
    bool use_xt = LAB_ENV("EMG3D_XT", 1) != 0;
    i64 xt_min_cells = LAB_ENV("EMG3D_XT_MIN", 8192);
    int th_lpw = (int)LAB_ENV("EMG3D_TH_LPW", 0);
    int force_lpw = (int)LAB_ENV("EMG3D_LPW", 0);
    bool use_twist = LAB_ENV("EMG3D_TWIST", 1) != 0;
    i64 twist_max_lines_env = LAB_ENV("EMG3D_TWIST_MAX", 0);
    int tw_stages = (int)LAB_ENV("EMG3D_TW_STAGES", 0);
    int use_split = (int)LAB_ENV("EMG3D_SPLIT", 2);
    i64 split_min_cells = LAB_ENV("EMG3D_SPLIT_MIN_CELLS", 2000000);
    int use_q = (int)LAB_ENV("EMG3D_Q", 1);
    i64 q_min_lines_env = LAB_ENV("EMG3D_Q_MIN_LINES", 0);
    int q_stages = (int)LAB_ENV("EMG3D_Q_STAGES", 0);
    int q_lpw = (int)LAB_ENV("EMG3D_Q_LPW", 0);
    int q_big_lab = (int)LAB_ENV("EMG3D_Q_BIG", 0);
    int use_qpl = (int)LAB_ENV("EMG3D_QPL", 7);
    i64 qpl_min_nl = LAB_ENV("EMG3D_QPL_MIN", 2);
    i64 qpl_max_nl = LAB_ENV("EMG3D_QPL_MAX_NL", 64);
    i64 qpl_m2_min = LAB_ENV("EMG3D_QPL_M2", 32);
    int qpl_chain_seg = (int)LAB_ENV("EMG3D_QPL_CHAIN", 4);
    i64 qpl_few_lines_env = LAB_ENV("EMG3D_QPL_FEW", 0);
    i64 qpl_max_lines = LAB_ENV("EMG3D_QPL_MAX", (i64)1 << 40);
    int use_qdesc = (int)LAB_ENV("EMG3D_QDESC", 1);
    i64 qdesc_max_threads_env = LAB_ENV("EMG3D_QDESC_MAX", 0);
    int fuse_max_seg = (int)LAB_ENV("EMG3D_QPL_FUSE", 4);
    i64 fuse_own = LAB_ENV("EMG3D_QPL_FUSE_W", 0);
    i64 fuse_max_bytes = LAB_ENV("EMG3D_QPL_FUSE_BYTES", (i64)64 << 20);
    int use_tha = (int)LAB_ENV("EMG3D_THA", 3);
    i64 tha_min_nl = LAB_ENV("EMG3D_THA_MIN", 33), tha_mid_nl = LAB_ENV("EMG3D_THA_MID", 64), tha_min_lines_env = LAB_ENV("EMG3D_THA_MIN_LINES", 0);
    i64 tha_max_nl = LAB_ENV("EMG3D_THA_MAX", 128);
    i64 tha_big_max_lines_env = LAB_ENV("EMG3D_THA_BIG_LINES", 0);
    int tha_split = (int)LAB_ENV("EMG3D_THA_SPLIT", 0);

    i64 q_min_lines() const { return q_min_lines_env > 0 ? q_min_lines_env : 8 * simds; }
    i64 twist_max_lines() const { return twist_max_lines_env > 0 ? twist_max_lines_env : q_min_lines(); }
    i64 qpl_few_lines() const { return qpl_few_lines_env > 0 ? qpl_few_lines_env : simds; }
    i64 qdesc_max_threads() const { return qdesc_max_threads_env > 0 ? qdesc_max_threads_env : (9000 * simds + 1023) / 1024; }
    i64 tha_min_lines() const { return tha_min_lines_env > 0 ? tha_min_lines_env : (1100 * simds + 1023) / 1024; }
    i64 tha_big_max_lines() const { return tha_big_max_lines_env > 0 ? tha_big_max_lines_env : (i64)SWEEP_THA_LPW * (simds / 4); }
};

struct SweepShape {
    i64 nC[3];
    int tsize;
    i64 cells() const { return nC[0] * nC[1] * nC[2]; }
    i64 edges() const {
        return nC[0] * (nC[1] + 1) * (nC[2] + 1) + (nC[0] + 1) * nC[1] * (nC[2] + 1) + (nC[0] + 1) * (nC[1] + 1) * nC[2];
    }
    i64 lines(int dir) const { return (nC[dir == 0 ? 1 : 0] / 2) * (nC[dir == 2 ? 1 : 2] / 2); }
    i64 lines_tot(int dir) const { return (nC[dir == 0 ? 1 : 0] - 1) * (nC[dir == 2 ? 1 : 2] - 1); }
    i64 field_stride(int c, int ax, bool transposed) const {
        const i64 d0 = (c == 0) ? nC[0] : nC[0] + 1, d1 = (c == 1) ? nC[1] : nC[1] + 1;
        return ax == 2 ? d0 * d1 : ((ax == 0) != transposed) ? 1 : (transposed ? d1 : d0);
    }
    i64 cell_stride(int ax, bool transposed) const {
        return ax == 2 ? nC[0] * nC[1] : ((ax == 0) != transposed) ? 1 : (transposed ? nC[1] : nC[0]);
    }
};

enum class SweepFamily { tpl, rp, qc, qc_big, thm, tha, qpl, qpl_chain };

inline void sweep_kernel_name(char* out, size_t len, SweepFamily f, int tsize, int p1 = 0, int p2 = 0) {
    static const char* const base[] = {"k_line_sweep", "k_line_sweep_rp", "k_line_sweep_qc", "k_line_sweep_qc_big", "k_line_sweep_thm",
                                       "k_line_sweep_tha", "k_line_sweep_qpl", "k_line_sweep_qpl_chain"};
    const char* tn = tsize == 16 ? "c128" : "f64";
    if (f == SweepFamily::tpl) snprintf(out, len, "%s<%s>", base[(int)f], tn);
    else if (f == SweepFamily::rp || f == SweepFamily::tha) snprintf(out, len, "%s<%s,%d>", base[(int)f], tn, p1);
    else snprintf(out, len, "%s<%s,%d,%d>", base[(int)f], tn, p1, p2);
}

struct SweepPlan {
    SweepFamily family = SweepFamily::tpl;
    int stages = 0, inst_lpw = 0, helpers = 0, NW = 0, M = 0, seg = 0;
    int qlpw = 0;
    bool big = false;
    bool split = false;
    bool xt = false;
    int work_id = 0;
    int fac_kind = 0;
    i64 fac_entries = 0;
    i64 mid = 0;
    bool qdesc = false;
    i64 nmax = 0;
    i64 lpw = 0;
    i64 rounds = 0;
    char name[64] = "";
};

inline bool sweep_wide_fits(const SweepKnobs& K, const SweepShape& G) {
    const i64 lim = (i64)1 << 32;
    const i64 mx = std::max(G.lines_tot(0), std::max(G.lines_tot(1), G.lines_tot(2)));
    return K.sweep_kernel == 0 && mx * 15 * (i64)G.tsize < lim && G.cells() * 8 < lim;
}
inline bool sweep_q_big_lines(const SweepKnobs& K, const SweepShape& G) {
    for (int d = 0; d < 3; ++d) if (G.lines(d) < std::max<i64>(K.q_min_lines(), 1)) return false;
    return K.order == 1 && K.use_q >= 1;
}
inline bool sweep_q_big(const SweepKnobs& K, const SweepShape& G) {
    return sweep_wide_fits(K, G) && sweep_q_big_lines(K, G) && (K.q_big_lab || G.edges() * (i64)G.tsize >= ((i64)1 << 32));
}
inline bool sweep_rp_fits(const SweepKnobs& K, const SweepShape& G) {
    return sweep_wide_fits(K, G) && G.edges() * (i64)G.tsize < ((i64)1 << 32) && !(K.q_big_lab && sweep_q_big_lines(K, G));
}
inline bool sweep_split_on(const SweepKnobs& K, const SweepShape& G) {
    return (K.use_split == 1 || (K.use_split == 2 && K.order == 1 && G.cells() >= K.split_min_cells)) &&
           (sweep_rp_fits(K, G) || sweep_q_big(K, G));
}

inline int sweep_tha_helpers(const SweepKnobs& K, const SweepShape& G, int dir) {
    if ((K.use_tha != 3 && K.use_tha != 2) || K.order != 1 || K.sweep_kernel != 0 || !K.use_twist || !sweep_rp_fits(K, G)) return 0;
// ... 26 lines not shown
    i64 mxs = 15 * G.lines_tot(dir) * (i64)G.tsize;
    for (int c = 0; c < 3; ++c) mxs = std::max(mxs, G.field_stride(c, dir, transposed) * (i64)G.tsize);
    mxs = std::max(mxs, G.cell_stride(dir, transposed) * 8);
    const i64 fac_bytes = 15 * G.lines_tot(dir) * G.nC[dir] * (i64)G.tsize;
    return mxs < lim24 && G.nC[dir] < lim24 && fac_bytes < ((i64)1 << 32);
}
inline int sweep_balanced_lpw(const SweepKnobs& K, i64 lines) {
    const i64 rounds = std::max<i64>(1, (lines + 16 * K.simds - 1) / (16 * K.simds));
    const i64 lpw = (lines + K.simds * rounds - 1) / (K.simds * rounds);
    return (int)std::min<i64>(16, std::max<i64>(lpw, 8));
}

inline SweepPlan plan_sweep(const SweepKnobs& K, const SweepShape& G, int dir) {
    SweepPlan p;
    const i64 nL = G.nC[dir], nmax = G.lines(dir), S = K.simds;
    const bool rp_fits = sweep_rp_fits(K, G), qpl = sweep_qpl_on(K, G, dir);
    p.nmax = nmax;
    p.split = sweep_split_on(K, G);
    p.xt = dir == 0 && K.use_xt && G.cells() >= K.xt_min_cells && !qpl;
    p.work_id = p.split ? (dir == 0 ? 0 : 1) : (p.xt ? 2 : 3 + dir);
    p.big = sweep_q_big(K, G) && !rp_fits;
    p.helpers = sweep_tha_helpers(K, G, dir);
    const bool q_on = K.use_q >= 2 || (K.use_q == 1 && nmax >= K.q_min_lines());
    p.fac_kind = (!qpl && sweep_twist_ok(K, G, dir, q_on, p.xt)) ? 3 : (!qpl && (rp_fits || p.big) && q_on) ? 4 : 0;
    p.mid = p.fac_kind == 3 ? (nL - 1) / 2 : nL - 1;
    p.fac_entries = (p.fac_kind == 4 ? 11 : 15) * nL;
    int p1 = 0, p2 = 0;
    if (p.fac_kind == 3 && p.helpers) {
        p.family = SweepFamily::tha;
        p1 = p.helpers;
        p.lpw = SWEEP_THA_LPW; p.rounds = (((nmax + p.lpw - 1) / p.lpw) * K.nsys + S / 4 - 1) / (S / 4);
    } else if (p.fac_kind == 3) {
        p.family = SweepFamily::thm;
        const i64 lines = nmax * K.nsys, r8 = (2 * ((lines + 7) / 8) + S - 1) / S, r12 = (2 * ((lines + 11) / 12) + S - 1) / S;
        p.inst_lpw = (K.th_lpw == 4 || K.th_lpw == 8 || K.th_lpw == 12) ? K.th_lpw : (23 * r12 < 20 * r8) ? 12 : 8;
        p.stages = K.tw_stages ? K.tw_stages : 3;
        p1 = p.stages; p2 = p.inst_lpw;
        p.lpw = p.inst_lpw; p.rounds = (2 * ((nmax + p.lpw - 1) / p.lpw) * K.nsys + S - 1) / S;
    } else if (qpl) {
        p.M = (nL >= K.qpl_m2_min) ? 2 : 1;
        p.seg = 4; while (p.seg < (nL + p.M - 1) / p.M) p.seg *= 2;
        p.NW = p.seg <= 16 ? 1 : p.seg / 16;
        p.family = (p.NW == 1 && p.M == 1 && K.order == 1 && p.seg <= K.qpl_chain_seg) ? SweepFamily::qpl_chain : SweepFamily::qpl;
        p1 = p.NW; p2 = p.M;
        p.fac_entries = 15 * (i64)p.M * p.seg;
        p.lpw = (16 * p.NW) / p.seg; p.rounds = (((nmax + p.lpw - 1) / p.lpw) * p.NW * K.nsys + S - 1) / S;
        p.qdesc = K.use_qdesc && K.order == 1 && p.NW == 1 && G.lines_tot(dir) * p.fac_entries < ((i64)1 << 32) &&
                  ((nmax + p.lpw - 1) / p.lpw) * 64 <= K.qdesc_max_threads();
    } else if ((rp_fits || p.big) && p.fac_kind == 4) {
        p.family = p.big ? SweepFamily::qc_big : SweepFamily::qc;
        p.inst_lpw = p.big ? 16 : K.q_lpw ? K.q_lpw : (nmax >= K.q_min_lines() ? 16 : 4);
        p.stages = (K.q_stages == 2 || K.q_stages == 3) ? K.q_stages
                 : (p.inst_lpw == 16 && nmax * K.nsys > 15 * S && nmax * K.nsys <= 16 * S) ? 2 : 3;
        p.qlpw = p.inst_lpw == 16 ? sweep_balanced_lpw(K, nmax * K.nsys) : p.inst_lpw;
        p1 = p.stages; p2 = p.inst_lpw;
        p.lpw = p.qlpw; p.rounds = (((nmax + p.lpw - 1) / p.lpw) * K.nsys + S - 1) / S;
    } else if (rp_fits || p.big) {
        p.family = SweepFamily::rp;
        p.lpw = K.force_lpw ? K.force_lpw : (nmax >= 8 * S ? 8 : 4);
        p.inst_lpw = (p.lpw == 8 || p.lpw == 12) ? (int)p.lpw : 4;
        p1 = p.inst_lpw;
        p.rounds = (((nmax + p.lpw - 1) / p.lpw) * K.nsys + S - 1) / S;
    } else {
        p.family = SweepFamily::tpl;
        p.lpw = 64; p.rounds = (((nmax + 63) / 64) * K.nsys + S - 1) / S;
    }
    sweep_kernel_name(p.name, sizeof p.name, p.family, G.tsize, p1, p2);
    return p;
}

constexpr int SWEEP_FUSE_MAX_PASSES = 16;
#if defined(__HIPCC__)
#define SWEEP_HD __host__ __device__
#else
#define SWEEP_HD
#endif
struct FuseGeom { int nX, own, nslabs, npass; };
SWEEP_HD inline int fuse_x0(const FuseGeom& g, int k) { return 1 + k * g.own; }
SWEEP_HD inline int fuse_x1(const FuseGeom& g, int k) { const int x = 1 + (k + 1) * g.own; return (k == g.nslabs - 1 || x > g.nX) ? g.nX : x; }
SWEEP_HD inline int fuse_lo(const FuseGeom& g, int k, int p) { const int v = fuse_x0(g, k) - (g.npass - 1 - p); return v < 1 ? 1 : v; }
SWEEP_HD inline int fuse_hi(const FuseGeom& g, int k, int p) { const int v = fuse_x1(g, k) + (g.npass - 1 - p); return v > g.nX - 1 ? g.nX - 1 : v; }
SWEEP_HD inline int fuse_owner(const FuseGeom& g, int j) { const int k = j <= 0 ? 0 : (j - 1) / g.own; return k > g.nslabs - 1 ? g.nslabs - 1 : k; }

struct FusePlan {
    bool fused = false;
    int axis = 0;
    int nw = 0;
    FuseGeom g = {0, 0, 0, 0};
    i64 scratch_bytes = 0;
};
inline void sweep_axes(int dir, int& P, int& Q) { P = dir == 0 ? 1 : 0; Q = dir == 2 ? 1 : 2; }
inline FusePlan plan_fuse(const SweepKnobs& K, const SweepShape& G, int dir, int npass) {
    FusePlan f;
    const SweepPlan p = plan_sweep(K, G, dir);
    if (K.order != 1 || (p.family != SweepFamily::qpl && p.family != SweepFamily::qpl_chain) || p.NW != 1 || p.M != 1 || !p.qdesc) return f;
    if (p.seg > K.fuse_max_seg || p.seg > 8 || npass < 3 || npass > SWEEP_FUSE_MAX_PASSES) return f;
#ifndef EMG3D_LAB
    if (p.family != SweepFamily::qpl_chain) return f;
#endif
    int P, Q;
    sweep_axes(dir, P, Q);
    f.axis = G.nC[Q] > G.nC[P] ? 1 : 0;
    const i64 nX = G.nC[f.axis ? Q : P];
    if (nX < 2 || nX > (1 << 20)) return f;
    i64 own = K.fuse_own > 0 ? K.fuse_own : 2;
    own = std::min<i64>(own, nX - 1);
    f.g.nX = (int)nX; f.g.own = (int)own; f.g.nslabs = (int)((nX - 1 + own - 1) / own); f.g.npass = npass;
    f.nw = p.family == SweepFamily::qpl_chain ? 8 : 4;
    f.scratch_bytes = (i64)K.nsys * f.g.nslabs * G.edges() * (i64)G.tsize;
    f.fused = f.scratch_bytes <= K.fuse_max_bytes;
    return f;
}
```

### emg3d_amd/csrc/sweep_qpl.hip

```cpp
#include "sweep_launch.hpp"
#ifndef EMG3D_UNIT_T
#define EMG3D_UNIT_T 2
#endif
#include "smooth_qpl.hpp"

template <class T, int NW, int M>
static void qpl_launch_c(dim3 grid, hipStream_t st, const LineArgs<T>& a) {
    hipLaunchKernelGGL((k_line_sweep_qpl<T, NW, M>), grid, dim3(64 * NW), 0, st, a);
}
template <class T, int NW>
static void qpl_launch_hl(dim3 grid, hipStream_t st, const LineArgs<T>& a) {
    hipLaunchKernelGGL((k_line_sweep_qpl<T, NW, 1, true>), grid, dim3(64 * NW), 0, st, a);
}
template <class T, int M>
static void qpl_launch_m(int nw, int dm, bool chain, dim3 grid, hipStream_t st, const LineArgs<T>& a) {
    if constexpr (M == 1) {
        if (chain && dm != 1 && nw == 1) {
            if (dm == 2) hipLaunchKernelGGL((k_line_sweep_qpl<T, 1, 1, false, 2, true>), grid, dim3(64), 0, st, a);
            else hipLaunchKernelGGL((k_line_sweep_qpl<T, 1, 1, false, 0, true>), grid, dim3(64), 0, st, a);
            return;
        }
    }
    if (dm == 1) hipLaunchKernelGGL((k_line_sweep_qpl<T, 1, M, false, 1>), grid, dim3(64), 0, st, a);
    else if (dm == 2) hipLaunchKernelGGL((k_line_sweep_qpl<T, 1, M, false, 2>), grid, dim3(64), 0, st, a);
    else if (nw == 1) qpl_launch_c<T, 1, M>(grid, st, a);
    else if (nw == 2) qpl_launch_c<T, 2, M>(grid, st, a);
    else if (nw == 4) qpl_launch_c<T, 4, M>(grid, st, a);
    else qpl_launch_c<T, 8, M>(grid, st, a);
}
template <class T>
void qpl_launch(int nw, int m, bool hl, int dm, bool chain, dim3 grid, hipStream_t st, const LineArgs<T>& a) {
    if (hl) {
        if (nw == 1) qpl_launch_hl<T, 1>(grid, st, a);
        else if (nw == 2) qpl_launch_hl<T, 2>(grid, st, a);
        else if (nw == 4) qpl_launch_hl<T, 4>(grid, st, a);
        else qpl_launch_hl<T, 8>(grid, st, a);
    } else if (m == 2) qpl_launch_m<T, 2>(nw, dm, false, grid, st, a);
    else qpl_launch_m<T, 1>(nw, dm, chain, grid, st, a);
}
template <class T>
void qpl_fused_launch(bool chain, dim3 grid, hipStream_t st, const LineArgs<T>& a) {
#ifdef EMG3D_LAB
    if (!chain) { hipLaunchKernelGGL((k_line_sweep_qpl<T, 4, 1, false, 2, false, true>), grid, dim3(256), 0, st, a); return; }
#endif
    hipLaunchKernelGGL((k_line_sweep_qpl<T, 8, 1, false, 2, true, true>), grid, dim3(512), 0, st, a);
}
#if EMG3D_UNIT_T != 1
template void qpl_launch<double>(int, int, bool, int, bool, dim3, hipStream_t, const LineArgs<double>&);
template void qpl_fused_launch<double>(bool, dim3, hipStream_t, const LineArgs<double>&);
#endif
#if EMG3D_UNIT_T != 0
template void qpl_launch<c128>(int, int, bool, int, bool, dim3, hipStream_t, const LineArgs<c128>&);
template void qpl_fused_launch<c128>(bool, dim3, hipStream_t, const LineArgs<c128>&);
#endif
```

### include/emg3d_hip.h

```cpp
#ifndef EMG3D_HIP_H
#define EMG3D_HIP_H

#include <stdint.h>

#ifdef __cplusplus
extern "C" {
#endif

#define EMG3D_HIP_ABI_VERSION 111
int emg3d_hip_version(void);
int emg3d_hip_device_count(int* count);
int emg3d_hip_set_device(int device);
int emg3d_hip_device_info(int device, char* name, int64_t* total_mem, int* cu_count);
int emg3d_hip_mem_info(int device, int64_t* free_bytes, int64_t* total_bytes);

int64_t emg3d_hip_release_cached(void);
int64_t emg3d_hip_cached_bytes(void);
int64_t emg3d_hip_cached_bytes_on(int device);


int emg3d_amat_x(int dtype, int64_t nx, int64_t ny, int64_t nz, void* r, const void* e,
                 const void* eta_x, const void* eta_y, const void* eta_z, const double* zeta,
                 const double* hx, const double* hy, const double* hz);

int emg3d_get_h_field(int dtype, int64_t nx, int64_t ny, int64_t nz, void* hfield, const void* efield,
                      const double* zeta, const double* hx, const double* hy, const double* hz,
                      double smu0_re, double smu0_im);

int emg3d_gauss_seidel(int dtype, int dir, int64_t nx, int64_t ny, int64_t nz, void* e,
                       const void* s, const void* eta_x, const void* eta_y, const void* eta_z,
                       const double* zeta, const double* hx, const double* hy, const double* hz,
                       int nu, int order);

int emg3d_restrict(int dtype, int64_t nx, int64_t ny, int64_t nz, int64_t cnx, int64_t cny,
                   int64_t cnz, void* cr, const void* r, const double* const* w, int sc_dir);

int emg3d_restrict_weights(const double* vectorN, const double* vectorCC, const double* h,
                           int64_t nh, const double* cvectorN, const double* cvectorCC,
                           const double* ch, int64_t n, double* wl, double* w0, double* wr);

int emg3d_solve(int dtype, void* amat, void* bvec, int64_t n);

int emg3d_blocks_to_amat(int dtype, void* amat, void* bvec, int64_t n, const void* middle,
                         const double* left, const void* rhs, int64_t im, int64_t nC);

int emg3d_prolongation(int dtype, int64_t nx, int64_t ny, int64_t nz, const double* hx,
                       const double* hy, const double* hz, const double* origin, void* e,
                       const void* ce, int sc_dir);

int emg3d_restrict_model(int is_complex, int64_t nx, int64_t ny, int64_t nz, void* cparam,
                         const void* param, int sc_dir);

int emg3d_sweep_plan(int dtype, int64_t nx, int64_t ny, int64_t nz, int dir, int order, int nsys, int cu_count, char* name,
                     int64_t* info);

int emg3d_sweep_fuse_plan(int dtype, int64_t nx, int64_t ny, int64_t nz, int dir, int order, int nsys, int cu_count, int npass, int own,
                          int max_seg, int64_t budget, int64_t* info, int64_t* ranges, int64_t nranges);

typedef struct emg3d_mg emg3d_mg_t;

int emg3d_mg_create(emg3d_mg_t** out, int dtype, int64_t nx, int64_t ny, int64_t nz,
                    const double* hx, const double* hy, const double* hz, const double* origin,
                    const void* eta_x, const void* eta_y, const void* eta_z, const double* zeta,
                    int device);
int emg3d_mg_create_sv(emg3d_mg_t** out, int dtype, int64_t nx, int64_t ny, int64_t nz, const double* hx,
                       const double* hy, const double* hz, const double* origin, const double* sv_x,
                       const double* sv_y, const double* sv_z, const double* zeta, double smu0_re,
                       double smu0_im, int device);

int emg3d_mg_create_vs(emg3d_mg_t** out, int dtype, int64_t nx, int64_t ny, int64_t nz, const double* hx,
                       const double* hy, const double* hz, const double* origin, const double* sigma_x,
                       const double* sigma_y, const double* sigma_z, const double* vol, const double* zeta,
                       double smu0_re, double smu0_im, int map, int device);
int emg3d_mg_create_vse(emg3d_mg_t** out, int dtype, int64_t nx, int64_t ny, int64_t nz, const double* hx,
                        const double* hy, const double* hz, const double* origin, const double* sigma_x,
                        const double* sigma_y, const double* sigma_z, const double* vol, const double* zeta,
                        const double* epsilon_r, double smu0_re, double smu0_im, double seps0, int map, int device);
void emg3d_mg_destroy(emg3d_mg_t* mg);

int emg3d_mg_set_params(emg3d_mg_t* mg, int cycle, int nu_init, int nu_pre, int nu_coarse,
                        int nu_post, const int* clevel, int order);

int emg3d_mg_set_sfield(emg3d_mg_t* mg, const void* sfield_host);
int emg3d_mg_set_sfield_vector(emg3d_mg_t* mg, const double* vector, double smu0_re, double smu0_im);
int emg3d_mg_set_sfield_dipole(emg3d_mg_t* mg, const double* src6, const double* scale6, int decimals,
                               int accumulate, double* sums3);
int emg3d_source_field(int dtype, int64_t nx, int64_t ny, int64_t nz, const double* hx, const double* hy,
                       const double* hz, const double* origin, const double* src6, const double* scale6,
                       int decimals, void* sfield, double* sums3);
int emg3d_mg_set_efield(emg3d_mg_t* mg, const void* efield_host);
int emg3d_mg_get_efield(emg3d_mg_t* mg, void* efield_host);
int emg3d_mg_get_residual(emg3d_mg_t* mg, void* rfield_host);
int emg3d_mg_get_hfield(emg3d_mg_t* mg, int use_zeta, double smu0_re, double smu0_im, void* hfield_host);

int emg3d_interp3d(int dtype, int64_t nx, int64_t ny, int64_t nz, const double* px, const double* py,
                   const double* pz, const void* values, int64_t n, const double* xi, int method, int has_fill,
                   double fill_value, double cval, void* out);
int emg3d_get_receiver_response(int dtype, int64_t nx, int64_t ny, int64_t nz, const double* hx, const double* hy,
                                const double* hz, const double* origin, const void* field, int is_electric,
                                int64_t n, const double* xyz, const double* factors, void* resp);
int emg3d_mg_get_receiver_response(emg3d_mg_t* mg, int magnetic, int use_zeta, double smu0_re, double smu0_im,
                                   int64_t n, const double* xyz, const double* factors, void* resp);

int emg3d_edges2cellaverages(int dtype, int64_t nx, int64_t ny, int64_t nz, const void* field, const double* vol,
                             void* out_x, void* out_y, void* out_z);
int emg3d_mg_gradient(emg3d_mg_t* mg, int efield_vec, double smu0_re, double smu0_im, double* grad);
int emg3d_mg_gradient3(emg3d_mg_t* mg, int efield_vec, double smu0_re, double smu0_im, double* grad_x, double* grad_y,
                       double* grad_z);

int emg3d_mg_grad_acc_reset(emg3d_mg_t* mg);
int emg3d_mg_grad_acc_add(emg3d_mg_t* mg, int fwd_bvec, double smu0_re, double smu0_im, const int32_t* use);
int emg3d_mg_grad_acc_get(emg3d_mg_t* mg, double* out);
int emg3d_mg_grad_acc3_reset(emg3d_mg_t* mg);
int emg3d_mg_grad_acc3_add(emg3d_mg_t* mg, int fwd_bvec, double smu0_re, double smu0_im, const int32_t* use);
int emg3d_mg_grad_acc3_get(emg3d_mg_t* mg, double* out_x, double* out_y, double* out_z);

int emg3d_cells2edges(int dtype, int64_t nx, int64_t ny, int64_t nz, const void* vx, const void* vy, const void* vz,
                      const double* vol, void* out_x, void* out_y, void* out_z);
int emg3d_mg_jvec_source(emg3d_mg_t* mg, int efield_vec, double smu0_re, double smu0_im, const double* vx, const double* vy,
                         const double* vz);
int emg3d_mg_jvec_source_b(emg3d_mg_t* mg, int fwd_bvec, double smu0_re, double smu0_im, const double* vx, const double* vy,
                           const double* vz, const int32_t* use);
int emg3d_mg_get_receiver_response_linear(emg3d_mg_t* mg, int64_t n, const double* xyz, const double* factors, void* resp);
int emg3d_mg_set_receiver_adjoint(emg3d_mg_t* mg, int64_t n, const double* xyz, const double* factors, const void* w,
                                  int accumulate);
int emg3d_mg_get_receiver_response_linear_h(emg3d_mg_t* mg, double smu0_re, double smu0_im, int64_t n, const double* xyz,
                                            const double* factors, void* resp);
int emg3d_mg_set_receiver_adjoint_ex(emg3d_mg_t* mg, int method, int magnetic, double smu0_re, double smu0_im, int64_t n,
                                     const double* xyz, const double* factors, const void* w, int accumulate);
int emg3d_mg_set_receiver_adjoint_b(emg3d_mg_t* mg, int method, int magnetic, double smu0_re, double smu0_im, int64_t n,
                                    const double* xyz, const double* factors, const void* w, const int32_t* use, int accumulate);
int emg3d_receiver_adjoint(int dtype, int64_t nx, int64_t ny, int64_t nz, const double* hx, const double* hy, const double* hz,
                           const double* origin, int is_electric, int method, double smu0_re, double smu0_im, int64_t n,
                           const double* xyz, const double* factors, const void* w, void* field);

int emg3d_volume_average_weights(const double* x1, int64_t n1, const double* x2, int64_t n2, double* w, int64_t* idx_in,
                                 int64_t* idx_out, int64_t* ptr, int64_t* nseg);
int emg3d_volume_average(int dtype, int64_t nx, int64_t ny, int64_t nz, const double* edges_x, const double* edges_y,
                         const double* edges_z, const void* values, int64_t mx, int64_t my, int64_t mz,
                         const double* new_edges_x, const double* new_edges_y, const double* new_edges_z, void* new_values,
// ... 71 lines not shown
```

Baseline: 252.5.

## Keep fused multi-pass sweep slab resident in LDS with precomputed image offsets

In the fused multi-pass line-sweep kernel (chain form), each workgroup's slab of the field is now copied into dynamic LDS when it fits (about 63 KiB). The passes then read and write that LDS image rather than global memory, using per-line image offsets computed once by a new small kernel and stored after the descriptors. It also adds an optional prefetch variant (lab only), a planning API that reports LDS eligibility, and caching of per-pass descriptor data across the fused passes. This targets the global-memory traffic between passes, at the cost of higher LDS use per workgroup, which can lower occupancy, plus an extra setup kernel and gather/scatter between global memory and LDS.

New measurement: 253.4 (median of 6 runs). No clear change (+0.4%).

```diff
diff --git a/emg3d_amd/_lib.py b/emg3d_amd/_lib.py
--- a/emg3d_amd/_lib.py
+++ b/emg3d_amd/_lib.py
@@ -13,7 +13,7 @@
 c_double = ctypes.c_double
 c_dp = ctypes.POINTER(ctypes.c_double)
 
-ABI_VERSION = 111
+ABI_VERSION = 112
 
 SIGNATURES = {
     "emg3d_hip_version": (c_int, []),
@@ -38,6 +38,8 @@
     "emg3d_sweep_plan": (c_int, [c_int, c_i64, c_i64, c_i64, c_int, c_int, c_int, c_int, ctypes.c_char_p, ctypes.POINTER(c_i64)]),
     "emg3d_sweep_fuse_plan": (c_int, [c_int, c_i64, c_i64, c_i64, c_int, c_int, c_int, c_int, c_int, c_int, c_int, c_i64, ctypes.POINTER(c_i64),
                                       ctypes.POINTER(c_i64), c_i64]),
+    "emg3d_sweep_fuse_lds": (c_int, [c_int, c_i64, c_i64, c_i64, c_int, c_int, c_int, c_int, c_int, c_int, c_int, c_i64, ctypes.POINTER(c_i64),
+                                     ctypes.POINTER(c_i64), c_i64, ctypes.POINTER(c_i64)]),
     "emg3d_mg_create": (c_int, [ctypes.POINTER(c_vp), c_int, c_i64, c_i64, c_i64, c_vp, c_vp, c_vp, c_vp,
                                 c_vp, c_vp, c_vp, c_vp, c_int]),
     "emg3d_mg_destroy": (None, [c_vp]),
@@ -249,3 +251,19 @@
             out["slabs"].append({"own": (r[0], r[1]), "edges": (r[2], r[3]),
                                  "live": [(r[4 + 2 * p], r[5 + 2 * p]) for p in range(int(npass))]})
     return out
+
+
+def sweep_fuse_lds(vnC, direction, npass, dtype=np.complex128, ordering='colour', nsys=1, cu_count=0, own=0, max_seg=0, lds_budget=-1,
+                   level_offsets=None):
+    info = (c_i64 * 6)()
+    n = 0 if level_offsets is None else len(level_offsets)
+    lev = (c_i64 * max(n, 1))(*([int(v) for v in level_offsets] if n else [0]))
+    img = (c_i64 * max(n, 1))()
+    check(load().emg3d_sweep_fuse_lds(dtype_code(dtype), int(vnC[0]), int(vnC[1]), int(vnC[2]), int(direction),
+                                      1 if ordering == 'colour' else 0, int(nsys), int(cu_count), int(npass), int(own), int(max_seg),
+                                      int(lds_budget), info, lev if n else None, n, img if n else None), "emg3d_sweep_fuse_lds")
+    out = {"fused": bool(info[0]), "lds": bool(info[1]), "prefetch": bool(info[2]), "lds_bytes": info[3], "plane": info[4],
+           "budget": info[5]}
+    if n and out["fused"]:
+        out["image_offsets"] = np.array(img[:n], dtype=np.int64)
+    return out
diff --git a/emg3d_amd/csrc/emg3d_hip.hip b/emg3d_amd/csrc/emg3d_hip.hip
--- a/emg3d_amd/csrc/emg3d_hip.hip
+++ b/emg3d_amd/csrc/emg3d_hip.hip
@@ -542,6 +542,29 @@
 }
 
 template <class T>
+static int fuse_lds_impl(i64 nx, i64 ny, i64 nz, int dir, int order, int nsys, int cu_count, int npass, int own, int max_seg, i64 lds_budget,
+                         int64_t* info, const int64_t* level_off, i64 n, int64_t* image_off) {
+    SweepKnobs K;
+    if (cu_count > 0) K.simds = 4 * (i64)cu_count;
+    else sweep_device_knobs<T>(K, current_device());
+    K.order = order; K.nsys = nsys;
+    if (own > 0) K.fuse_own = own;
+    if (max_seg > 0) K.fuse_max_seg = max_seg;
+    if (lds_budget >= 0) K.fuse_lds_bytes = std::min<i64>(lds_budget, SWEEP_FUSE_LDS_MAX);
+    const SweepShape G{{nx, ny, nz}, (int)sizeof(T)};
+    const FusePlan f = plan_fuse(K, G, dir - 1, npass);
+    info[0] = f.fused ? 1 : 0; info[1] = f.lds ? 1 : 0; info[2] = f.prefetch ? 1 : 0; info[3] = f.lds_bytes; info[4] = f.im.plane;
+    info[5] = K.fuse_lds_bytes;
+    if (!f.fused || !level_off || !image_off) return 0;
+    const FuseOffMap m = fuse_off_map(f.im, dir - 1, f.axis, G.nC);
+    for (i64 i = 0; i < n; ++i) {
+        if (level_off[i] < 0 || level_off[i] >= G.edges()) return -2;
+        image_off[i] = fuse_image_offset(m, (unsigned)level_off[i]);
+    }
+    return 0;
+}
+
+template <class T>
 static int jvec_stage(MG<T>* m, const double* const hv[3], const double* dv[3]) {
     Level<T>& L = *m->lv0;
     double* stage = reinterpret_cast<double*>(L.r);
@@ -879,6 +902,13 @@
                  : fuse_plan_impl<double>(nx, ny, nz, dir, order, nsys, cu_count, npass, own, max_seg, budget, info, ranges, nranges);
 }
 
+int emg3d_sweep_fuse_lds(int dtype, int64_t nx, int64_t ny, int64_t nz, int dir, int order, int nsys, int cu_count, int npass, int own,
+                         int max_seg, int64_t lds_budget, int64_t* info, const int64_t* level_off, int64_t n, int64_t* image_off) {
+    if (nx < 2 || ny < 2 || nz < 2 || dir < 1 || dir > 3 || order < 0 || order > 1 || nsys < 1 || nsys > 64 || npass < 0 || !info || n < 0) return -2;
+    return dtype ? fuse_lds_impl<c128>(nx, ny, nz, dir, order, nsys, cu_count, npass, own, max_seg, lds_budget, info, level_off, n, image_off)
+                 : fuse_lds_impl<double>(nx, ny, nz, dir, order, nsys, cu_count, npass, own, max_seg, lds_budget, info, level_off, n, image_off);
+}
+
 int emg3d_mg_create(emg3d_mg_t** out, int dtype, int64_t nx, int64_t ny, int64_t nz, const double* hx,
                     const double* hy, const double* hz, const double* origin, const void* eta_x,
                     const void* eta_y, const void* eta_z, const double* zeta, int device) {
diff --git a/emg3d_amd/csrc/mg.hpp b/emg3d_amd/csrc/mg.hpp
--- a/emg3d_amd/csrc/mg.hpp
+++ b/emg3d_amd/csrc/mg.hpp
@@ -51,6 +51,7 @@
     unsigned qdn[3][4] = {{0, 0, 0, 0}, {0, 0, 0, 0}, {0, 0, 0, 0}};
     T* fz[3] = {nullptr, nullptr, nullptr};
     i64 fz_n[3] = {0, 0, 0};
+    bool fso[3][4] = {{false, false, false, false}, {false, false, false, false}, {false, false, false, false}};
     FusePlan fuse[3];
     int fuse_key[3] = {-1, -1, -1};
     std::vector<int> passes[3];
@@ -1132,7 +1133,7 @@
             if (n <= 0) continue;
             const unsigned grid = xcd_grid((n + lpg - 1) / lpg);
             const i64 nthreads = (i64)grid * 64;
-            void* tab = try_alloc<char>(nthreads * a.qM * (3 * 16 + 8 * 16));
+            void* tab = try_alloc<char>(nthreads * a.qM * (i64)QPL_DESC_BYTES + (a.qM == 1 ? nthreads * (i64)QPL_FSO_BYTES : 0));
             if (!tab) return;
             a.qd = tab; a.qdn = (unsigned)nthreads;
             if (!broken) qpl_launch<T>(1, a.qM, false, 1, false, dim3(grid), stream, a);
@@ -1368,6 +1369,20 @@
             if (L.fz[dir]) release(L.fz[dir]);
             L.fz[dir] = z; L.fz_n[dir] = need;
         }
+        if (F.lds) {
+            for (int c : seq) {
+                if (L.fso[dir][c]) continue;
+                const i64 n = L.qdn[dir][c];
+                FuseOffArgs o;
+                o.qd = L.qd[dir][c]; o.out = (char*)L.qd[dir][c] + n * (i64)QPL_DESC_BYTES; o.qdn = (unsigned)n;
+                o.m = fuse_off_map(F.im, dir, F.axis, L.nC);
+                for (int q = 0; q < 3; ++q) if ((i64)o.m.off[q] != L.fl.off[q]) F.lds = false;
+                if (!F.lds) break;
+                if (!broken) qpl_fuse_offsets_launch(o, stream);
+                L.fso[dir][c] = true;
+            }
+            check_launch();
+        }
         return F;
     }
     void smooth_fused(Level<T>& L, int dir, const SweepPlan& P, const FusePlan& F, const std::vector<int>& seq, const LineArgs<T>& a) {
@@ -1378,11 +1393,16 @@
         b.fseq = 0;
         for (int p = 0; p < F.g.npass; ++p) b.fseq |= (unsigned long long)seq[(size_t)p] << (4 * p);
         for (int c = 0; c < 4; ++c) { b.fqd[c] = L.qd[dir][c]; b.fqdn[c] = L.qd[dir][c] ? L.qdn[dir][c] : 0u; }
-        if (log_launches) fprintf(stderr, "[sweep] nC %lld %lld %lld L %d lines %lld kernel %s split %d fused passes %d slabs %d own %d\n", (long long)a.nC[0],
-                                  (long long)a.nC[1], (long long)a.nC[2], a.L, (long long)a.nLinesTot, P.name, a.split, F.g.npass, F.g.nslabs, F.g.own);
+        int fv = (F.lds ? 1 : 0) | (F.prefetch ? 2 : 0);
+#ifndef EMG3D_LAB
+        fv &= 1;
+#endif
+        if (log_launches) fprintf(stderr, "[sweep] nC %lld %lld %lld L %d lines %lld kernel %s split %d fused passes %d slabs %d own %d slab %s %lld B%s\n",
+                                  (long long)a.nC[0], (long long)a.nC[1], (long long)a.nC[2], a.L, (long long)a.nLinesTot, P.name, a.split, F.g.npass,
+                                  F.g.nslabs, F.g.own, (fv & 1) ? "in LDS" : "in global memory", (long long)F.lds_bytes, (fv & 2) ? " prefetch" : "");
         memcpy(sweep_name, P.name, sizeof sweep_name);
         if (broken) return;
-        qpl_fused_launch<T>(P.family == SweepFamily::qpl_chain, bgrid((unsigned)F.g.nslabs), stream, b);
+        qpl_fused_launch<T>(P.family == SweepFamily::qpl_chain, fv, (fv & 1) ? (size_t)F.lds_bytes : 0, bgrid((unsigned)F.g.nslabs), stream, b);
         ScatterArgs sa;
         sa.nE = L.nE; sa.g = F.g;
         int Pa, Qa;
@@ -1711,7 +1731,7 @@
         auto clear = [](Level<T>& L) {
             for (int d = 0; d < 3; ++d) {
                 L.fac[d] = nullptr; L.fac_kind[d] = 0; L.plan_key[d] = -1; L.fuse_key[d] = -1;
-                for (int c = 0; c < 4; ++c) { L.qd[d][c] = nullptr; L.qdn[d][c] = 0; }
+                for (int c = 0; c < 4; ++c) { L.qd[d][c] = nullptr; L.qdn[d][c] = 0; L.fso[d][c] = false; }
             }
         };
         if (lv0) clear(*lv0);
diff --git a/emg3d_amd/csrc/smooth.hpp b/emg3d_amd/csrc/smooth.hpp
--- a/emg3d_amd/csrc/smooth.hpp
+++ b/emg3d_amd/csrc/smooth.hpp
@@ -54,6 +54,8 @@
     i64 cntA, cntB;
     i64 t, jQ0, cnt;
 };
+constexpr unsigned QPL_DESC_BYTES = 3 * 16 + 8 * 16, QPL_FSO_BYTES = 20;
+static_assert(sizeof(LineArgs<double>) == 720 && sizeof(LineArgs<c128>) == 720, "LineArgs grew: see the note at its end");
 
 template <class T>
 __device__ __forceinline__ bool line_of_thread(const LineArgs<T>& a, i64& jP, i64& jQ) {
diff --git a/emg3d_amd/csrc/smooth_qpl.hpp b/emg3d_amd/csrc/smooth_qpl.hpp
--- a/emg3d_amd/csrc/smooth_qpl.hpp
+++ b/emg3d_amd/csrc/smooth_qpl.hpp
@@ -48,11 +48,26 @@
                  "s"(a.rs.nP), "s"(a.rs.nQ), "s"(a.qd), "s"(a.qdn));
 }
 
-template <class T, int NW, int M, bool HL = false, int DM = 0, bool CH = false, bool FZ = false>
+template <class T>
+__device__ __forceinline__ void qpl_fused_args_burst(const LineArgs<T>& a) {
+    asm volatile("" :: "s"(a.fe), "s"(a.fnE), "s"(a.fax), "s"(a.fnX), "s"(a.fown), "s"(a.fns), "s"(a.fnp), "s"(a.fseq));
+}
+
+struct QplWords { uint4 u0, u1, u2; };
+struct QplCoef { emg_d2 cf[8]; };
+template <class T>
+struct QplStatic { T S, S0; uint4 so; unsigned so8; };
+template <class T>
+struct QplRows { T W0[5], Wr[5]; };
+extern __shared__ __align__(16) unsigned char qpl_image_[];
+
+template <class T, int NW, int M, bool HL = false, int DM = 0, bool CH = false, bool FZ = false, int FV = 0>
 __global__ __launch_bounds__(64 * NW) void k_line_sweep_qpl(LineArgs<T> a) {
     static_assert(DM == 0 || (!HL && (NW == 1 || FZ)), "descriptors: one wave per workgroup, colour order");
     static_assert(!CH || ((NW == 1 || FZ) && M == 1 && !HL), "chain form: lines inside one wave, one block per quad");
     static_assert(!FZ || (DM == 2 && M == 1 && !HL), "fused passes: descriptors, one block per quad, colour order");
+    static_assert(FV == 0 || (FZ && CH), "LDS-resident slab / prefetch: the chain form of the fused loop");
+    constexpr bool LD = (FV & 1) != 0, PF = (FV & 2) != 0;
     constexpr int NQ = 16 * NW;
 #ifdef EMG3D_LAB
     long long qts[7] = {0, 0, 0, 0, 0, 0, 0};
@@ -62,6 +77,7 @@
 #endif
     QPL_TS(0);
     qpl_args_burst(a);
+    if constexpr (FZ) qpl_fused_args_burst(a);
     QPL_TS(1);
     const int tid = threadIdx.x;
     const int quad = tid >> 2, r = tid & 3;
@@ -76,7 +92,10 @@
     const void* qd_ = a.qd;
     u32 qdn_ = a.qdn;
     u32 tix = (u32)wg * (64u * NW) + (u32)tid;
-    auto one = [&](const u32 gline, const u32 nlines, const u32 t_, const u32 jQ0_) {
+    T* const img = reinterpret_cast<T*>(qpl_image_);
+    u32 img_ra = 0;
+    auto one = [&](const u32 gline, const u32 nlines, const u32 t_, const u32 jQ0_, const QplWords* pw, const QplStatic<T>* ps, const QplCoef* pc,
+                   const QplRows<T>* pr, auto&& mid, auto&& late) {
     const bool live = gline < nlines;
     const int nL = (int)a.rs.nL;
     auto ld_d = [](const double* base, u32 idx) -> double { return *reinterpret_cast<const double*>(reinterpret_cast<const char*>(base) + idx * 8u); };
@@ -88,6 +107,7 @@
     double av[M][4], dv[M][4];
     bool lastb[M], inl[M];
     u32 dS[M], dS0[M];
+    u32 iS[M], iS0[M];
     constexpr int QD_U4 = 3, QD_D2 = 8;
     if constexpr (DM == 2) {
         const uint4* const q4 = reinterpret_cast<const uint4*>(qd_);
@@ -96,10 +116,16 @@
         emg_d2 cf[M][QD_D2];
 #pragma unroll
         for (int j = 0; j < M; ++j) {
+            if constexpr (FZ) {
+                u[j][0] = pw->u0; u[j][1] = pw->u1; u[j][2] = pw->u2;
+#pragma unroll
+                for (int k = 0; k < QD_D2; ++k) cf[j][k] = pc->cf[k];
+            } else {
 #pragma unroll
             for (int k = 0; k < QD_U4; ++k) u[j][k] = q4[(u32)(QD_U4 * j + k) * qdn_ + tix];
 #pragma unroll
             for (int k = 0; k < QD_D2; ++k) cf[j][k] = c2[(u32)(QD_D2 * j + k) * qdn_ + tix];
+            }
         }
         QPL_TS(2);
         T E[M][6], S[M], E0[M], S0[M];
@@ -108,6 +134,24 @@
             const u32 oE[6] = {u[j][0].x, u[j][0].y, u[j][0].z, u[j][0].w, u[j][1].x, u[j][1].y};
             dS[j] = u[j][1].z; dS0[j] = u[j][2].x;
             inl[j] = (u[j][2].z & 1u) != 0; lastb[j] = (u[j][2].z & 2u) != 0;
+            if constexpr (FZ) {
+#pragma unroll
+                for (int c = 0; c < 5; ++c) { W0[j][c] = pr->W0[c]; Wr[j][c] = pr->Wr[c]; }
+                S[j] = ps->S; S0[j] = ps->S0;
+                if constexpr (LD) {
+                    const uint4 so = ps->so;
+                    const u32 iE[6] = {(so.x & 0xffffu) - img_ra, (so.x >> 16) - img_ra, (so.y & 0xffffu) - img_ra, (so.y >> 16) - img_ra,
+                                       (so.z & 0xffffu) - img_ra, (so.z >> 16) - img_ra};
+                    iS[j] = (so.w >> 16) - img_ra; iS0[j] = (ps->so8 & 0xffffu) - img_ra;
+#pragma unroll
+                    for (int t = 0; t < 6; ++t) E[j][t] = img[iE[t]];
+                    E0[j] = img[(so.w & 0xffffu) - img_ra];
+                } else {
+#pragma unroll
+                    for (int t = 0; t < 6; ++t) E[j][t] = ld_t(e, oE[t]);
+                    E0[j] = ld_t(e, u[j][1].w);
+                }
+            } else {
             const T* w = a.fac + u[j][2].y;
 #pragma unroll
             for (int c = 0; c < 5; ++c) W0[j][c] = w[(u32)(wpk(0, c) * (M * seg))];
@@ -122,6 +166,7 @@
             S[j] = ld_t(s, dS[j]);
             E0[j] = ld_t(e, u[j][1].w);
             S0[j] = ld_t(s, dS0[j]);
+            }
         }
 #pragma unroll
         for (int j = 0; j < M; ++j) {
@@ -411,6 +456,7 @@
     }
 
     QPL_TS(4);
+    mid();
     auto bwd_row = [&](int j) {
         const double ar = (r == 0) ? av[j][0] : (r == 1) ? av[j][1] : (r == 2) ? av[j][2] : av[j][3];
         const double dr = (r == 0) ? dv[j][0] : (r == 1) ? dv[j][1] : (r == 2) ? dv[j][2] : dv[j][3];
@@ -463,6 +509,7 @@
     for (int k = 0; k < 4; ++k) v[k] = (ch + 1 < seg) ? xb[p][quad + 1][k][0] : Zero<T>::v();
     }
     QPL_TS(5);
+    late();
     T* eo = ebase;
 #pragma unroll
     for (int j = M - 1; j >= 0; --j) {
@@ -471,8 +518,13 @@
         for (int l = 0; l < 4; ++l) { cmsc(x0, W0[j][l + 1], v[l]); cmsc(xr, Wr[j][l + 1], v[l]); }
         const int i = ch * M + j;
         if (live && inl[j]) {
+            if constexpr (LD) {
+                if (r == 0) img[iS0[j]] = x0;
+                if (!lastb[j]) img[iS[j]] = xr;
+            } else {
             if (r == 0) eo[dS0[j]] = x0;
             if (!lastb[j]) eo[dS[j]] = xr;
+            }
         }
         if (j > 0) {
             const double ar = (r == 0) ? av[j][0] : (r == 1) ? av[j][1] : (r == 2) ? av[j][2] : av[j][3];
@@ -488,59 +540,177 @@
     if constexpr (FZ) {
         const FuseGeom g{a.fnX, a.fown, a.fns, a.fnp};
         const int k = (int)wg;
+        const int ra = fuse_lo(g, k, 0) - 1, rb = fuse_hi(g, k, 0) + 1;
+        u32 fpb[3], fps;
         {
-            T* __restrict__ dst = ebase;
-            const T* __restrict__ src = a.e + boff_;
-            const int ra = fuse_lo(g, k, 0) - 1, rb = fuse_hi(g, k, 0) + 1;
+            const u32 nO_ = a.fax ? a.rs.nP : a.rs.nQ, nL_ = a.rs.nL;
+            const u32 bO = nL_ * (nO_ + 1u), bX = bO + (nL_ + 1u) * nO_;
+            fpb[0] = 0u; fpb[1] = a.fax ? bO : bX; fpb[2] = a.fax ? bX : bO;
+            fps = bX + (nL_ + 1u) * (nO_ + 1u);
+        }
+        img_ra = (u32)ra * fps;
+        auto for_edges = [&](const int ia, const int ib, auto&& fn) {
             const int X = a.fax ? 2 : 1;
             const u32 nO = a.fax ? a.rs.nP : a.rs.nQ;
 #pragma unroll
             for (int c = 0; c < 3; ++c) {
                 const u32 dL = a.rs.nL + (c != 0 ? 1u : 0u), dX = (u32)g.nX + (c != X ? 1u : 0u), dO = nO + ((c == 0 || c == X) ? 1u : 0u);
-                const int rbc = rb < (int)dX - 1 ? rb : (int)dX - 1;
-                if (rbc < ra) continue;
-                const u32 w = (u32)(rbc - ra + 1);
+                const int ibc = ib < (int)dX - 1 ? ib : (int)dX - 1;
+                if (ibc < ia) continue;
+                const u32 w = (u32)(ibc - ia + 1);
                 const u32 stL = a.rs.st[c][0], stX = a.fax ? a.rs.st[c][2] : a.rs.st[c][1], stO = a.fax ? a.rs.st[c][1] : a.rs.st[c][2];
                 const bool xf = stX < stL;
                 const u32 n0 = xf ? w : dL, n1 = xf ? dL : w, tot = n0 * n1 * dO;
                 for (u32 idx = (u32)tid; idx < tot; idx += 64u * NW) {
                     const u32 t = idx / n0, i0 = idx - t * n0, i2 = t / n1, i1 = t - i2 * n1;
-                    const u32 iX = (u32)ra + (xf ? i0 : i1), iL = xf ? i1 : i0;
-                    const u32 off = a.rs.off[c] + iL * stL + iX * stX + i2 * stO;
-                    dst[off] = src[off];
+                    const u32 iX = (u32)ia + (xf ? i0 : i1), iL = xf ? i1 : i0;
+                    fn(a.rs.off[c] + iL * stL + iX * stX + i2 * stO, LD ? (iX - (u32)ra) * fps + fpb[c] + iL + dL * i2 : 0u);
                 }
             }
-        }
-        __threadfence_block();
+        };
+        {
+            T* __restrict__ dst = ebase;
+            const T* __restrict__ src = a.e + boff_;
+            for_edges(ra, rb, [&](const u32 off, const u32 io) { if constexpr (LD) img[io] = src[off]; else dst[off] = src[off]; });
+        }
+        if constexpr (!LD) __threadfence_block();
         __syncthreads();
-        const u32 lslot = (u32)(quad >> lseg), wslot0 = (u32)(((tid >> 6) * 16) >> lseg);
-        for (int p = 0; p < g.npass; ++p) {
-            const int c = (int)((a.fseq >> (4 * p)) & 3ull);
+        const u32 lslot = (u32)(quad >> lseg), wslot0 = (u32)__builtin_amdgcn_readfirstlane((int)(((tid >> 6) * 16) >> lseg));
+        const u32 r1 = (u32)r + 1u, tri1 = (r1 * (r1 + 1u)) >> 1;
+        auto row_entry = [&](const u32 i) -> u32 { return i <= r1 ? tri1 + i : ((i * (i + 1u)) >> 1) + r1; };
+        auto pass_lines = [&](const int p, int& c, u32& qa, u32& nx, u32& cA) -> u32 {
+            c = (int)((a.fseq >> (4 * p)) & 3ull);
             const int cP = c & 1, cQ = c >> 1;
-            const u32 cA = (u32)a.nA[cP], cB = (u32)a.nB2[cQ];
+            cA = (u32)a.nA[cP];
+            const u32 cB = (u32)a.nB2[cQ];
             const int cX = a.fax ? cQ : cP;
-            const u32 qa = (u32)(fuse_lo(g, k, p) - cX) >> 1, qb = (u32)(fuse_hi(g, k, p) + 1 - cX) >> 1;
-            const u32 nx = qb > qa ? qb - qa : 0u;
-            const u32 nloc = nx * (a.fax ? cA : cB);
-            qd_ = a.fqd[c]; qdn_ = a.fqdn[c];
-            for (u32 base = 0; base < nloc; base += (u32)lpg) {
-                if (base + wslot0 < nloc) {
-                    const u32 m = base + lslot;
-                    const bool lv = m < nloc;
-                    const u32 mm = lv ? m : base + wslot0;
-                    u32 qq, bq;
-                    if (a.fax == 0) { bq = mm / nx; qq = qa + (mm - bq * nx); }
-                    else { const u32 t = mm / cA; qq = mm - t * cA; bq = qa + t; }
-                    const u32 gl = bq * cA + qq;
-                    tix = ((gl >> (4 - lseg)) << 6) + ((((gl & ((16u >> lseg) - 1u)) << lseg) + (u32)ch) << 2) + (u32)r;
-                    one(lv ? 0u : 1u, 1u, 0u, 0u);
+            qa = (u32)(fuse_lo(g, k, p) - cX) >> 1;
+            const u32 qb = (u32)(fuse_hi(g, k, p) + 1 - cX) >> 1;
+            nx = qb > qa ? qb - qa : 0u;
+            return nx * (a.fax ? cA : cB);
+        };
+        auto line_thread = [&](const u32 base, const u32 nloc, const u32 qa, const u32 nx, const u32 cA, bool& lv) -> u32 {
+            const u32 m = base + lslot;
+            lv = m < nloc;
+            const u32 mm = lv ? m : base + wslot0;
+            u32 qq, bq;
+            if (a.fax == 0) { bq = mm / nx; qq = qa + (mm - bq * nx); }
+            else { const u32 t = mm / cA; qq = mm - t * cA; bq = qa + t; }
+            const u32 gl = bq * cA + qq;
+            return ((gl >> (4 - lseg)) << 6) + ((((gl & ((16u >> lseg) - 1u)) << lseg) + (u32)ch) << 2) + (u32)r;
+        };
+        auto at = [](const void* base, const u32 byte) -> const char* { return reinterpret_cast<const char*>(base) + byte; };
+        auto fetch_words = [&](const int c, const u32 t) -> QplWords {
+            const void* const q4 = a.fqd[c];
+            const u32 n = a.fqdn[c];
+            QplWords w;
+            if constexpr (LD) w.u0 = make_uint4(0u, 0u, 0u, 0u);
+            else w.u0 = *reinterpret_cast<const uint4*>(at(q4, t * 16u));
+            w.u1 = *reinterpret_cast<const uint4*>(at(q4, (n + t) * 16u)); w.u2 = *reinterpret_cast<const uint4*>(at(q4, (2u * n + t) * 16u));
+            return w;
+        };
+        auto fetch_coef = [&](const int c, const u32 t) -> QplCoef {
+            const u32 n = a.fqdn[c];
+            const void* const q4 = a.fqd[c];
+            QplCoef q;
+#pragma unroll
+            for (int i = 0; i < 8; ++i) q.cf[i] = *reinterpret_cast<const emg_d2*>(at(q4, ((u32)(3 + i) * n + t) * 16u));
+            return q;
+        };
+        auto fetch_rows = [&](const QplWords& w) -> QplRows<T> {
+            QplRows<T> q;
+            auto fac = [&](const u32 byte) -> T {
+                if constexpr (FV == 0) return *reinterpret_cast<const T*>(at(a.fac + w.u2.y, byte));
+                else return *reinterpret_cast<const T*>(at(a.fac, w.u2.y * (u32)sizeof(T) + byte));
+            };
+#pragma unroll
+            for (int i = 0; i < 5; ++i) q.W0[i] = fac((u32)(wpk(0, i) * seg) * (u32)sizeof(T));
+#pragma unroll
+            for (int i = 0; i < 5; ++i) q.Wr[i] = fac((row_entry((u32)i) * (u32)seg) * (u32)sizeof(T));
+            return q;
+        };
+        auto fetch_static = [&](const int c, const u32 t, const QplWords& w) -> QplStatic<T> {
+            const u32 n = a.fqdn[c];
+            QplStatic<T> q;
+            const T* const sb = a.s + boff_;
+            q.S = *reinterpret_cast<const T*>(at(sb, w.u1.z * (u32)sizeof(T)));
+            q.S0 = *reinterpret_cast<const T*>(at(sb, w.u2.x * (u32)sizeof(T)));
+            if constexpr (LD) {
+                q.so = *reinterpret_cast<const uint4*>(at(a.fqd[c], n * QPL_DESC_BYTES + t * 16u));
+                q.so8 = *reinterpret_cast<const unsigned*>(at(a.fqd[c], n * (QPL_DESC_BYTES + 16u) + t * 4u));
+            } else { q.so = make_uint4(0u, 0u, 0u, 0u); q.so8 = 0u; }
+            return q;
+        };
+        if constexpr (!PF) {
+            for (int p = 0; p < g.npass; ++p) {
+                int c;
+                u32 qa, nx, cA;
+                const u32 nloc = pass_lines(p, c, qa, nx, cA);
+                for (u32 base = 0; base < nloc; base += (u32)lpg) {
+                    if (base + wslot0 < nloc) {
+                        bool lv;
+                        const u32 t = line_thread(base, nloc, qa, nx, cA, lv);
+                        const QplWords w = fetch_words(c, t);
+                        const QplCoef kf = fetch_coef(c, t);
+                        const QplStatic<T> q = fetch_static(c, t, w);
+                        const QplRows<T> rw = fetch_rows(w);
+                        one(lv ? 0u : 1u, 1u, 0u, 0u, &w, &q, &kf, &rw, [] {}, [] {});
+                    }
                 }
-            }
-            __threadfence_block();
-            __syncthreads();
+                if constexpr (!LD) __threadfence_block();
+                __syncthreads();
+            }
+        } else {
+            auto seek = [&](int& p, u32& base) {
+                while (p < g.npass) {
+                    int c;
+                    u32 qa, nx, cA;
+                    if (base + wslot0 < pass_lines(p, c, qa, nx, cA)) return;
+                    ++p; base = 0;
+                }
+            };
+            auto words_of = [&](const int p, const u32 base, int& c, u32& t, bool& lv) -> QplWords {
+                u32 qa, nx, cA;
+                const u32 nloc = pass_lines(p, c, qa, nx, cA);
+                t = line_thread(base, nloc, qa, nx, cA, lv);
+                return fetch_words(c, t);
+            };
+            int p0 = 0, done = 0;
+            u32 b0 = 0;
+            seek(p0, b0);
+            if (p0 < g.npass) {
+                int p1 = p0, c0, c1;
+                u32 b1 = b0 + (u32)lpg, t0, t1;
+                bool lv0, lv1;
+                seek(p1, b1);
+                QplWords w0 = words_of(p0, b0, c0, t0, lv0);
+                QplCoef k0 = fetch_coef(c0, t0);
+                QplStatic<T> q0 = fetch_static(c0, t0, w0);
+                QplRows<T> rw0 = fetch_rows(w0);
+                for (;;) {
+                    for (; done < p0; ++done) { if constexpr (!LD) __threadfence_block(); __syncthreads(); }
+                    const bool n1 = p1 < g.npass;
+                    const QplWords w1 = words_of(n1 ? p1 : p0, n1 ? b1 : b0, c1, t1, lv1);
+                    QplStatic<T> q1;
+                    QplCoef k1;
+                    QplRows<T> rw1;
+                    one(lv0 ? 0u : 1u, 1u, 0u, 0u, &w0, &q0, &k0, &rw0, [&] { k1 = fetch_coef(c1, t1); q1 = fetch_static(c1, t1, w1); },
+                        [&] { rw1 = fetch_rows(w1); });
+                    if (!n1) break;
+                    p0 = p1; b0 = b1; lv0 = lv1; w0 = w1; q0 = q1; k0 = k1; rw0 = rw1;
+                    b1 += (u32)lpg;
+                    seek(p1, b1);
+                }
+            }
+            for (; done < g.npass; ++done) { if constexpr (!LD) __threadfence_block(); __syncthreads(); }
+        }
+        if constexpr (LD) {
+            T* __restrict__ dst = ebase;
+            const int ea = k == 0 ? 0 : fuse_x0(g, k), eb = k == g.nslabs - 1 ? g.nX : fuse_x1(g, k) - 1;
+            for_edges(ea, eb, [&](const u32 off, const u32 io) { dst[off] = img[io]; });
         }
     } else if constexpr (!HL) {
-        one((u32)wg * (u32)lpg + (u32)(quad >> lseg), (u32)((a.mode == 0) ? a.cntA * a.cntB : a.cnt), (u32)a.t, (u32)a.jQ0);
+        one((u32)wg * (u32)lpg + (u32)(quad >> lseg), (u32)((a.mode == 0) ? a.cntA * a.cntB : a.cnt), (u32)a.t, (u32)a.jQ0, nullptr, nullptr, nullptr, nullptr, [] {}, [] {});
 #ifdef EMG3D_LAB
         if ((a.tile & 512) && blockIdx.x == 0 && threadIdx.x == 0) {
             asm volatile("s_waitcnt vmcnt(0)" ::: "memory");
@@ -561,7 +731,7 @@
             if (jq1 > nQm) jq1 = nQm;
             const int n = jq1 - jq0 + 1;
             for (int base = 0; base < n; base += lpg) {
-                one((u32)(quad >> lseg), (u32)min(n - base, lpg), (u32)tt, (u32)(jq0 + base));
+                one((u32)(quad >> lseg), (u32)min(n - base, lpg), (u32)tt, (u32)(jq0 + base), nullptr, nullptr, nullptr, nullptr, [] {}, [] {});
                 __threadfence_block();
                 __syncthreads();
             }
diff --git a/emg3d_amd/csrc/sweep_launch.hpp b/emg3d_amd/csrc/sweep_launch.hpp
--- a/emg3d_amd/csrc/sweep_launch.hpp
+++ b/emg3d_amd/csrc/sweep_launch.hpp
@@ -11,6 +11,13 @@
 template <class T> bool tha_attrs(int max_dyn_lds);
 
 template <class T> void qpl_launch(int nw, int m, bool hl, int dm, bool chain, dim3 grid, hipStream_t st, const LineArgs<T>& a);
-template <class T> void qpl_fused_launch(bool chain, dim3 grid, hipStream_t st, const LineArgs<T>& a);
+template <class T> void qpl_fused_launch(bool chain, int fv, size_t dyn_lds, dim3 grid, hipStream_t st, const LineArgs<T>& a);
+struct FuseOffArgs {
+    const void* qd;
+    void* out;
+    unsigned qdn;
+    FuseOffMap m;
+};
+void qpl_fuse_offsets_launch(const FuseOffArgs& a, hipStream_t st);
 
 template <class T> void residual_launch(int mode, int kz, dim3 grid, hipStream_t st, const ResidualArgs<T>& a);
diff --git a/emg3d_amd/csrc/sweep_plan.hpp b/emg3d_amd/csrc/sweep_plan.hpp
--- a/emg3d_amd/csrc/sweep_plan.hpp
+++ b/emg3d_amd/csrc/sweep_plan.hpp
@@ -23,6 +23,7 @@
     return (2 * SWEEP_THA_RING * 5 + 2 * ((nL + 1) / 2 + 2)) * (5 * SWEEP_THA_LPW) * (i64)tsize;
 }
 
+constexpr int SWEEP_FUSE_LDS_MAX = 63 * 1024;
 struct SweepKnobs {
     i64 simds = 1024;
     i64 lds_limit = 160 * 1024;
@@ -57,6 +58,8 @@
     int fuse_max_seg = (int)LAB_ENV("EMG3D_QPL_FUSE", 4);
     i64 fuse_own = LAB_ENV("EMG3D_QPL_FUSE_W", 0);
     i64 fuse_max_bytes = LAB_ENV("EMG3D_QPL_FUSE_BYTES", (i64)64 << 20);
+    i64 fuse_lds_bytes = std::min<i64>(LAB_ENV("EMG3D_QPL_FUSE_LDS_BYTES", SWEEP_FUSE_LDS_MAX), SWEEP_FUSE_LDS_MAX);
+    int fuse_prefetch = (int)LAB_ENV("EMG3D_QPL_FUSE_PREFETCH", 0);
     int use_tha = (int)LAB_ENV("EMG3D_THA", 3);
     i64 tha_min_nl = LAB_ENV("EMG3D_THA_MIN", 33), tha_mid_nl = LAB_ENV("EMG3D_THA_MID", 64), tha_min_lines_env = LAB_ENV("EMG3D_THA_MIN_LINES", 0);
     i64 tha_max_nl = LAB_ENV("EMG3D_THA_MAX", 128);
@@ -249,8 +252,61 @@
 SWEEP_HD inline int fuse_hi(const FuseGeom& g, int k, int p) { const int v = fuse_x1(g, k) + (g.npass - 1 - p); return v > g.nX - 1 ? g.nX - 1 : v; }
 SWEEP_HD inline int fuse_owner(const FuseGeom& g, int j) { const int k = j <= 0 ? 0 : (j - 1) / g.own; return k > g.nslabs - 1 ? g.nslabs - 1 : k; }
 
+struct FuseImage { i64 dL[3], dO[3], pb[3], plane, elems; };
+inline FuseImage fuse_image(const FuseGeom& g, int axis, i64 nL, i64 nO) {
+    FuseImage im;
+    const int X = axis ? 2 : 1, O = axis ? 1 : 2;
+    for (int c = 0; c < 3; ++c) {
+        im.dL[c] = nL + (c != 0 ? 1 : 0);
+        im.dO[c] = nO + ((c == 0 || c == X) ? 1 : 0);
+    }
+    im.pb[0] = 0; im.pb[O] = im.dL[0] * im.dO[0]; im.pb[X] = im.pb[O] + im.dL[O] * im.dO[O];
+    im.plane = im.pb[X] + im.dL[X] * im.dO[X];
+    im.elems = 0;
+    for (int k = 0; k < g.nslabs; ++k) {
+        const int ra = fuse_lo(g, k, 0) - 1, rb = fuse_hi(g, k, 0) + 1;
+        im.elems = std::max(im.elems, (i64)(rb - ra + 1) * im.plane - (rb > g.nX - 1 ? im.dL[X] * im.dO[X] : 0));
+    }
+    return im;
+}
+
+struct FuseOffMap {
+    unsigned plane, off[3], d0[3], d1[3], pb[3], dL[3];
+    int axL, axX, axO;
+};
+SWEEP_HD inline unsigned fuse_image_offset(const FuseOffMap& m, unsigned o) {
+    const int c = o >= m.off[2] ? 2 : o >= m.off[1] ? 1 : 0;
+#define FUSE_OF(v) (c == 0 ? (v)[0] : c == 1 ? (v)[1] : (v)[2])
+    const unsigned d0 = FUSE_OF(m.d0), d1 = FUSE_OF(m.d1);
+    const unsigned l = o - FUSE_OF(m.off), q = l / d0, i0 = l - q * d0, i2 = q / d1, i1 = q - i2 * d1;
+#define FUSE_ALONG(ax) ((ax) == 0 ? i0 : (ax) == 1 ? i1 : i2)
+    const unsigned v = FUSE_ALONG(m.axX) * m.plane + FUSE_OF(m.pb) + FUSE_ALONG(m.axL) + FUSE_OF(m.dL) * FUSE_ALONG(m.axO);
+#undef FUSE_ALONG
+#undef FUSE_OF
+    return v;
+}
+inline FuseOffMap fuse_off_map(const FuseImage& im, int dir, int axis, const i64 nC[3]) {
+    FuseOffMap m;
+    const int P = dir == 0 ? 1 : 0, Q = dir == 2 ? 1 : 2;
+    const int ax[3] = {dir, P, Q};
+    m.plane = (unsigned)im.plane;
+    i64 o = 0;
+    for (int q = 0; q < 3; ++q) {
+        m.pb[ax[q]] = (unsigned)im.pb[q]; m.dL[ax[q]] = (unsigned)im.dL[q];
+        m.off[q] = (unsigned)o;
+        m.d0[q] = (unsigned)(q == 0 ? nC[0] : nC[0] + 1); m.d1[q] = (unsigned)(q == 1 ? nC[1] : nC[1] + 1);
+        o += (i64)m.d0[q] * m.d1[q] * (q == 2 ? nC[2] : nC[2] + 1);
+    }
+    m.axL = dir; m.axX = axis ? Q : P; m.axO = axis ? P : Q;
+    return m;
+}
+
 struct FusePlan {
     bool fused = false;
+    bool lds = false;
+    bool prefetch = false;
+    i64 lds_bytes = 0;
+    FuseImage im = {{0, 0, 0}, {0, 0, 0}, {0, 0, 0}, 0, 0};
     int axis = 0;
     int nw = 0;
     FuseGeom g = {0, 0, 0, 0};
@@ -276,5 +332,9 @@
     f.nw = p.family == SweepFamily::qpl_chain ? 8 : 4;
     f.scratch_bytes = (i64)K.nsys * f.g.nslabs * G.edges() * (i64)G.tsize;
     f.fused = f.scratch_bytes <= K.fuse_max_bytes;
+    f.im = fuse_image(f.g, f.axis, G.nC[dir], G.nC[f.axis ? P : Q]);
+    f.lds_bytes = f.im.elems * (i64)G.tsize;
+    f.lds = f.fused && p.family == SweepFamily::qpl_chain && f.lds_bytes <= K.fuse_lds_bytes && (nX + 1) * f.im.plane < 65536;
+    f.prefetch = f.fused && p.family == SweepFamily::qpl_chain && K.fuse_prefetch != 0;
     return f;
 }
diff --git a/emg3d_amd/csrc/sweep_qpl.hip b/emg3d_amd/csrc/sweep_qpl.hip
--- a/emg3d_amd/csrc/sweep_qpl.hip
+++ b/emg3d_amd/csrc/sweep_qpl.hip
@@ -39,17 +39,36 @@
     else qpl_launch_m<T, 1>(nw, dm, chain, grid, st, a);
 }
 template <class T>
-void qpl_fused_launch(bool chain, dim3 grid, hipStream_t st, const LineArgs<T>& a) {
+void qpl_fused_launch(bool chain, int fv, size_t dyn_lds, dim3 grid, hipStream_t st, const LineArgs<T>& a) {
 #ifdef EMG3D_LAB
     if (!chain) { hipLaunchKernelGGL((k_line_sweep_qpl<T, 4, 1, false, 2, false, true>), grid, dim3(256), 0, st, a); return; }
+    if (fv == 3) { hipLaunchKernelGGL((k_line_sweep_qpl<T, 8, 1, false, 2, true, true, 3>), grid, dim3(512), dyn_lds, st, a); return; }
+    if (fv == 2) { hipLaunchKernelGGL((k_line_sweep_qpl<T, 8, 1, false, 2, true, true, 2>), grid, dim3(512), 0, st, a); return; }
 #endif
-    hipLaunchKernelGGL((k_line_sweep_qpl<T, 8, 1, false, 2, true, true>), grid, dim3(512), 0, st, a);
+    if (fv & 1) hipLaunchKernelGGL((k_line_sweep_qpl<T, 8, 1, false, 2, true, true, 1>), grid, dim3(512), dyn_lds, st, a);
+    else hipLaunchKernelGGL((k_line_sweep_qpl<T, 8, 1, false, 2, true, true>), grid, dim3(512), 0, st, a);
+}
+static __global__ __launch_bounds__(256) void k_fuse_offsets(FuseOffArgs a) {
+    const unsigned t = blockIdx.x * 256u + threadIdx.x;
+    if (t >= a.qdn) return;
+    const uint4* const q4 = reinterpret_cast<const uint4*>(a.qd);
+    const uint4 u0 = q4[t], u1 = q4[a.qdn + t], u2 = q4[2u * a.qdn + t];
+    auto img = [&](const unsigned o) -> unsigned { return fuse_image_offset(a.m, o); };
+    uint4 o;
+    o.x = img(u0.x) | (img(u0.y) << 16); o.y = img(u0.z) | (img(u0.w) << 16); o.z = img(u1.x) | (img(u1.y) << 16);
+    o.w = img(u1.w) | (img(u1.z) << 16);
+    uint4* const o4 = reinterpret_cast<uint4*>(a.out);
+    o4[t] = o;
+    reinterpret_cast<unsigned*>(o4 + a.qdn)[t] = img(u2.x);
+}
+void qpl_fuse_offsets_launch(const FuseOffArgs& a, hipStream_t st) {
+    hipLaunchKernelGGL(k_fuse_offsets, dim3((a.qdn + 255u) / 256u), dim3(256), 0, st, a);
 }
 #if EMG3D_UNIT_T != 1
 template void qpl_launch<double>(int, int, bool, int, bool, dim3, hipStream_t, const LineArgs<double>&);
-template void qpl_fused_launch<double>(bool, dim3, hipStream_t, const LineArgs<double>&);
+template void qpl_fused_launch<double>(bool, int, size_t, dim3, hipStream_t, const LineArgs<double>&);
 #endif
 #if EMG3D_UNIT_T != 0
 template void qpl_launch<c128>(int, int, bool, int, bool, dim3, hipStream_t, const LineArgs<c128>&);
-template void qpl_fused_launch<c128>(bool, dim3, hipStream_t, const LineArgs<c128>&);
+template void qpl_fused_launch<c128>(bool, int, size_t, dim3, hipStream_t, const LineArgs<c128>&);
 #endif
diff --git a/include/emg3d_hip.h b/include/emg3d_hip.h
--- a/include/emg3d_hip.h
+++ b/include/emg3d_hip.h
@@ -7,7 +7,7 @@
 extern "C" {
 #endif
 
-#define EMG3D_HIP_ABI_VERSION 111
+#define EMG3D_HIP_ABI_VERSION 112
 int emg3d_hip_version(void);
 int emg3d_hip_device_count(int* count);
 int emg3d_hip_set_device(int device);
@@ -56,6 +56,9 @@
 
 int emg3d_sweep_fuse_plan(int dtype, int64_t nx, int64_t ny, int64_t nz, int dir, int order, int nsys, int cu_count, int npass, int own,
                           int max_seg, int64_t budget, int64_t* info, int64_t* ranges, int64_t nranges);
+
+int emg3d_sweep_fuse_lds(int dtype, int64_t nx, int64_t ny, int64_t nz, int dir, int order, int nsys, int cu_count, int npass, int own,
+                         int max_seg, int64_t lds_budget, int64_t* info, const int64_t* level_off, int64_t n, int64_t* image_off);
 
 typedef struct emg3d_mg emg3d_mg_t;
 
```
